# zrlhahaha/Direct12PBRRenderer

Hardware: AMD Instinct MI355X
Metric: shaded Mpixel/s at 4K G-buffer (full deferred frame: clustered shade + bloom + auto-exposure + ACES) (higher is better)
Workload: dtype f32

## Files before the change

direct12pbrrenderer_amd/_lib.py:

```python
import ctypes as C
import os

from .structs import CubeF32, GBuffer, Global, HaloPeer, Texture2D, Tile, View

_HERE = os.path.dirname(os.path.abspath(__file__))
LIB_PATH = os.environ.get("PBR_HIP_LIB", os.path.join(_HERE, "libpbr_hip.so"))

_u32, _f32, _int, _vp, _sz = C.c_uint32, C.c_float, C.c_int, C.c_void_p, C.c_size_t

SIGNATURES = {
    "pbr_version": (C.c_char_p, []),
    "pbr_cube_texels": (_sz, [_u32, _u32]),
    "pbr_cube_mip_offset": (_sz, [_u32, _u32]),
    "pbr_env_padded_texels": (_sz, [_u32, _u32]),
    "pbr_env_padded_mip_offset": (_sz, [_u32, _u32]),
    "pbr_bloom_chain_texels": (_sz, [_u32, _u32]),
    "pbr_bloom_level_offset": (_sz, [_u32, _u32, _u32]),
    "pbr_ctx_create": (_int, [_int, C.POINTER(_vp)]),
    "pbr_ctx_destroy": (None, [_vp]),
    "pbr_ctx_set_stream": (_int, [_vp, _vp]),
    "pbr_ctx_use_own_stream": (_int, [_vp]),
    "pbr_ctx_get_stream": (_vp, [_vp]),
    "pbr_ctx_side_begin": (_int, [_vp]),
    "pbr_ctx_side_end": (_int, [_vp]),
    "pbr_ctx_side_join": (_int, [_vp]),
    "pbr_last_error": (C.c_char_p, [_vp]),
    "pbr_sync": (_int, [_vp]),
    "pbr_brdf_lut": (_int, [_vp, _u32, _vp]),
    "pbr_rgbe_decode": (_int, [_vp, _vp, C.c_size_t, _vp]),
    "pbr_cube_gen_mips": (_int, [_vp, _vp, _u32, _u32]),
    "pbr_prefilter_env": (_int, [_vp, C.POINTER(CubeF32), _u32, _u32, _vp]),
    "pbr_prefilter_env_mip": (_int, [_vp, C.POINTER(CubeF32), _u32, _u32, _f32, _vp]),
    "pbr_env_pad": (_int, [_vp, _vp, _u32, _u32, _vp]),
    "pbr_sh9_project": (_int, [_vp, C.POINTER(CubeF32), _vp]),
    "pbr_cluster_build": (_int, [_vp, C.POINTER(Global), _vp]),
    "pbr_cluster_cull": (_int, [_vp, C.POINTER(Global), _vp, _int, _vp]),
    "pbr_clustered": (_int, [_vp, C.POINTER(Global), _vp, _int, _vp]),
    "pbr_deferred_shade": (_int, [_vp, C.POINTER(Global), C.POINTER(Tile), C.POINTER(GBuffer),
                                  _vp, _u32, _vp, _u32, _u32, _vp, _vp, _int, _vp, _u32]),
    "pbr_deferred_shade_rects": (_int, [_vp, C.POINTER(Global), C.POINTER(Tile), C.POINTER(GBuffer),
                                        _vp, _u32, _vp, _u32, _u32, _vp, _vp, _int, _vp, _u32, _vp, _u32]),
    "pbr_deferred_shade_f32": (_int, [_vp, C.POINTER(Global), C.POINTER(Tile), C.POINTER(GBuffer),
                                      _vp, _u32, _vp, _u32, _u32, _vp, _vp, _int, _vp, _u32]),
    "pbr_lut_fold_x": (_int, [_vp, _vp, _u32, _vp]),
    "pbr_deferred_shade_folded": (_int, [_vp, C.POINTER(Global), C.POINTER(Tile), C.POINTER(GBuffer),
                                         _vp, _u32, _vp, _u32, _u32, _vp, _vp, _int, _vp, _u32]),
    "pbr_deferred_shade_rects_folded": (_int, [_vp, C.POINTER(Global), C.POINTER(Tile), C.POINTER(GBuffer),
                                               _vp, _u32, _vp, _u32, _u32, _vp, _vp, _int, _vp, _u32, _vp, _u32]),
    "pbr_skybox": (_int, [_vp, C.POINTER(Global), C.POINTER(Tile), C.POINTER(CubeF32), _vp, _u32, _vp, _u32]),
    "pbr_gbuffer_encode": (_int, [_vp, _vp, _vp, _vp, _u32, _u32, _u32, _vp, _vp, _vp]),
    "pbr_gbuffer_raster_scratch_bytes": (_sz, [_u32, _u32, _u32]),
    "pbr_gbuffer_raster_min_scratch_bytes": (_sz, [_u32, _u32, _u32]),
    "pbr_gbuffer_raster": (_int, [_vp, C.POINTER(Global), C.POINTER(Tile), _vp, _u32, _vp, _u32, _vp, _u32, _u32,
                                  _vp, _vp, _vp, _vp, _vp, _u32, _vp, _sz]),
    "pbr_texture2d_bytes": (_sz, [_u32, _u32, _u32, _u32]),
    "pbr_bc1_decode": (_int, [_vp, _vp, _u32, _u32, _u32, _u32, _vp]),
    "pbr_bc6h_chain_bytes": (_sz, [_u32, _u32]),
    "pbr_bc6h_decode_cube": (_int, [_vp, C.POINTER(_vp * 6), _u32, _u32, _vp]),
    "pbr_texture2d_gen_mips": (_int, [_vp, _vp, _u32, _u32, _u32, _u32]),
    "pbr_bc1_encode": (_int, [_vp, _vp, _u32, _u32, _u32, _u32, _vp]),
    "pbr_gbuffer_raster_textured_scratch_bytes": (_sz, [_u32, _u32, _u32]),
    "pbr_gbuffer_raster_textured_min_scratch_bytes": (_sz, [_u32, _u32, _u32]),
    "pbr_gbuffer_raster_textured": (_int, [_vp, C.POINTER(Global), C.POINTER(Tile), _vp, _u32, _vp, _u32, _vp, _u32, _u32,
                                           _vp, _vp, _vp, _vp, _vp, _u32, _vp, _sz, _vp, C.POINTER(Texture2D), _u32]),
    "pbr_bloom_prefilter": (_int, [_vp, _vp, _u32, _u32, _u32, _vp, _f32, _f32]),
    "pbr_blur_h": (_int, [_vp, _vp, _u32, _u32, _vp, _u32, _u32]),
    "pbr_blur_v": (_int, [_vp, _vp, _u32, _u32, _vp, _u32, _u32]),
    "pbr_bloom_upsample_add": (_int, [_vp, _vp, _u32, _u32, _vp, _u32, _u32, _vp]),
    "pbr_bloom_up_level": (_int, [_vp, _vp, _vp, _u32, _u32, _vp, _u32, _u32]),
    "pbr_bloom_merge": (_int, [_vp, _vp, _u32, _vp, _u32, _u32]),
    "pbr_bloom": (_int, [_vp, _vp, _u32, _u32, _u32, _vp, _vp, _f32, _f32]),
    "pbr_bloom_prefilter_rect": (_int, [_vp, _vp, _u32, _u32, _u32, _vp, _u32, _u32, _u32, C.POINTER(_u32 * 4), _f32, _f32]),
    "pbr_bloom_prefilter_rects": (_int, [_vp, _vp, _u32, _u32, _u32, _vp, _u32, _u32, _u32, _vp, _u32, _f32, _f32]),
    "pbr_bloom_tiled": (_int, [_vp, _vp, _u32, C.POINTER(_u32 * 4), _u32, _u32, _vp, _vp, C.POINTER(_u32 * 4), _f32, _f32, _vp]),
    "pbr_bloom_histogram": (_int, [_vp, _vp, _u32, _u32, _u32, _vp, _vp, _f32, _f32, C.POINTER(_u32 * 4), _f32, _f32, _vp]),
    "pbr_lum_histogram": (_int, [_vp, _vp, _u32, _u32, _u32, _f32, _f32, _vp]),
    "pbr_lum_average": (_int, [_vp, _vp, _u32, _f32, _f32, _f32, _vp]),
    "pbr_tonemap": (_int, [_vp, _vp, _u32, _u32, _u32, _vp, _vp, _u32]),
    "pbr_average_tonemap": (_int, [_vp, _vp, _u32, _f32, _f32, _f32, _vp, _vp, _vp, _vp, _u32, _u32, _u32, _vp, _u32]),
    "pbr_clustered_views": (_int, [_vp, C.POINTER(View), _u32]),
    "pbr_deferred_shade_views": (_int, [_vp, C.POINTER(View), _u32, _u32, _u32, _vp, _u32, _vp, _u32, _u32]),
    "pbr_bloom_histogram_views": (_int, [_vp, C.POINTER(View), _u32, _u32, _u32, _f32, _f32, _f32, _f32]),
    "pbr_lum_average_views": (_int, [_vp, C.POINTER(View), _u32, _u32, _f32, _f32]),
    "pbr_tonemap_views": (_int, [_vp, C.POINTER(View), _u32, _u32, _u32]),
    "pbr_comm_unique_id": (_int, [_vp]),
    "pbr_comm_init": (_int, [_vp, _int, _int, _vp]),
    "pbr_allreduce_hist": (_int, [_vp, _vp]),
    "pbr_halo_staging_bytes": (_sz, [C.POINTER(HaloPeer), _u32]),
    "pbr_halo_exchange": (_int, [_vp, _vp, _u32, _u32, C.POINTER(HaloPeer), _u32, _vp, _sz]),
    "pbr_halo_pack": (_int, [_vp, _vp, _u32, _u32, C.POINTER(HaloPeer), _u32, _vp, _sz, _int]),
    "pbr_runtime_error": (C.c_char_p, []),
    "pbr_runtime_mismatch_dirs": (_int, [C.c_char_p, C.c_char_p]),
    "pbr_membench_read": (_int, [_vp, _vp, _sz, _vp, _u32]),
    "pbr_valubench": (_int, [_vp, _u32, _u32, _u32, _vp]),
    "pbr_ctx_set_bloom_shader_order": (_int, [_vp, _int]),
}

KNOBS_ONLY = {
    "pbr_ctx_set_cu_masks": (_int, [_vp, _vp, _vp, _u32]),
}

_lib = None


def load():
    global _lib
    if _lib is not None:
        return _lib
    if not os.path.exists(LIB_PATH):
        raise RuntimeError(
            f"{LIB_PATH} not found: build it with `make -C direct12pbrrenderer_amd/csrc` "
            "(or __graft_entry__.build()).  There is no CPU fallback for the HIP path.")
    import torch
    lib = C.CDLL(LIB_PATH)
    for name, (res, args) in SIGNATURES.items():
        fn = getattr(lib, name)
        fn.restype = res
        fn.argtypes = args
    for name, (res, args) in KNOBS_ONLY.items():
        fn = getattr(lib, name, None)
        if fn is not None:
            fn.restype = res
            fn.argtypes = args
    _lib = lib
    return lib
```

direct12pbrrenderer_amd/api.py:

```python
import ctypes as C

import numpy as np
import torch

from . import _lib
from .structs import (Texture2D, BLOOM_KNEE, BLOOM_THRESHOLD, CLUSTER_DTYPE, ENV_MIPS, HISTOGRAM_BINS,
                      INV_LOG_LUMINANCE_RANGE, LIGHT_DTYPE, LOG_LUMINANCE_RANGE, MIN_LOG_LUMINANCE,
                      NUM_CLUSTERS, DRAW_DTYPE, DRAW_MAPS_DTYPE, TEX_BC1_BLOCKS, TEX_FORMATS, VERTEX_DTYPE, CubeF32, GBuffer, Global, HaloPeer, Tile, View, bloom_chain_texels, bc6h_chain_bytes, cube_texels, env_padded_texels, texture2d_bytes)


class PbrError(RuntimeError):
    pass


def _ptr(t):
    if t is None:
        return None
    if isinstance(t, torch.Tensor):
        if not t.is_cuda:
            raise PbrError("expected a device tensor")
        if not t.is_contiguous():
            raise PbrError("expected a contiguous tensor")
        return C.c_void_p(t.data_ptr())
    return C.c_void_p(int(t))


class PbrContext:

    def __init__(self, device=0, use_torch_stream=True):
        self.lib = _lib.load()
        self.device = int(device)
        h = C.c_void_p()
        st = self.lib.pbr_ctx_create(self.device, C.byref(h))
        if st != 0:
            raise PbrError(f"pbr_ctx_create({device}) failed: status {st}")
        self.h = h
        self.torch_device = torch.device("cuda", self.device)
        if use_torch_stream:
            self.bind_torch_stream()

    def bind_torch_stream(self):
        s = torch.cuda.current_stream(self.torch_device)
        self._check(self.lib.pbr_ctx_set_stream(self.h, C.c_void_p(s.cuda_stream)))

    def close(self):
        if getattr(self, "h", None):
            self.lib.pbr_ctx_destroy(self.h)
            self.h = None

    def __del__(self):
        try:
            self.close()
        except Exception:
            pass

    def _check(self, st):
        if st != 0:
            msg = self.lib.pbr_last_error(self.h)
            raise PbrError(f"status {st}: {msg.decode() if msg else '?'}")

    def side_begin(self):
        self._check(self.lib.pbr_ctx_side_begin(self.h))

    def side_end(self):
        self._check(self.lib.pbr_ctx_side_end(self.h))

    def side_join(self):
        self._check(self.lib.pbr_ctx_side_join(self.h))

    def sync(self):
        self._check(self.lib.pbr_sync(self.h))

    def use_own_stream(self):
        self._check(self.lib.pbr_ctx_use_own_stream(self.h))

    def set_bloom_shader_order(self, on):
        self._check(self.lib.pbr_ctx_set_bloom_shader_order(self.h, 1 if on else 0))

    def partition_cus(self, side_cus, total_cus=None, layout="low", allow_uneven=False):
        if not hasattr(self.lib, "pbr_ctx_set_cu_masks"):
            raise PbrError("partition_cus: pbr_ctx_set_cu_masks is an entry point of the knobs build only (PBR_HIP_LIB=.../libpbr_hip_knobs.so): "
                           "the CU partition is a measurement aid, not part of the product library (round 6)")
        if side_cus and layout == "low" and int(side_cus) % 32 and not allow_uneven:
            raise PbrError(f"partition_cus: layout 'low' takes a multiple of 32 compute units (got {side_cus}): an uneven share per XCD runs at the poorest XCD's pace")
        if not side_cus:
            self._check(self.lib.pbr_ctx_set_cu_masks(self.h, None, None, 0))
            return
        n = int(total_cus or torch.cuda.get_device_properties(self.torch_device).multi_processor_count)
        words = (n + 31) // 32
# ... 50 lines not shown
            self._check(self.lib.pbr_prefilter_env_mip(self.h, C.byref(c), size, m, float(m) / float(max(mips - 1, 1)), C.c_void_p(dst)))
        return out

    def env_pad(self, env, size, mips=ENV_MIPS, out=None):
        out = out if out is not None else self.empty((env_padded_texels(size, mips), 4), torch.float16)
        self._check(self.lib.pbr_env_pad(self.h, _ptr(env), size, mips, _ptr(out)))
        return out

    def bc6h_decode_cube(self, faces, size, mip_levels, out=None):
        faces = list(faces)
        if len(faces) != 6:
            raise PbrError(f"bc6h_decode_cube: six faces, got {len(faces)}")
        nbytes = bc6h_chain_bytes(size, mip_levels)
        for f in faces:
            if isinstance(f, torch.Tensor) and nbytes and f.numel() * f.element_size() != nbytes:
                raise PbrError(f"bc6h_decode_cube: a face of {f.numel() * f.element_size()} bytes, {size}^2 x {mip_levels} levels takes {nbytes}")
        ptrs = (C.c_void_p * 6)(*[_ptr(f) for f in faces])
        if out is None:
            if not nbytes:
                raise PbrError(f"bad BC6H cube description: {size}^2, {mip_levels} levels")
            out = self.empty((cube_texels(size, mip_levels), 4), torch.float32)
        self._check(self.lib.pbr_bc6h_decode_cube(self.h, C.byref(ptrs), int(size), int(mip_levels), _ptr(out)))
        return out

    def sh9_project(self, sky, sky_size, sky_mips=1, out=None):
        out = out if out is not None else self.empty((28,), torch.float32)
        c = CubeF32(sky.data_ptr(), sky_size, sky_mips)
        self._check(self.lib.pbr_sh9_project(self.h, C.byref(c), _ptr(out)))
        return out

    def alloc_clusters(self):
        return self.zeros((NUM_CLUSTERS * CLUSTER_DTYPE.itemsize,), torch.uint8)

    def cluster_build(self, g: Global, clusters):
        self._check(self.lib.pbr_cluster_build(self.h, C.byref(g), _ptr(clusters)))

    def cluster_cull(self, g: Global, lights, n, clusters):
        self._check(self.lib.pbr_cluster_cull(self.h, C.byref(g), _ptr(lights), int(n), _ptr(clusters)))

    def clustered(self, g: Global, lights, n, clusters):
        self._check(self.lib.pbr_clustered(self.h, C.byref(g), _ptr(lights), int(n), _ptr(clusters)))

    def deferred_shade(self, g: Global, tile: Tile, gb, pitch, lut, lut_res, env, env_size, env_mips,
                       clusters, lights, num_lights, hdr, hdr_pitch):
        s = GBuffer(gb["A"].data_ptr(), gb["B"].data_ptr(), gb["C"].data_ptr(), gb["depth"].data_ptr(),
                    gb["stencil"].data_ptr(), pitch)
        self._check(self.lib.pbr_deferred_shade(self.h, C.byref(g), C.byref(tile), C.byref(s), _ptr(lut), lut_res,
                                                _ptr(env), env_size, env_mips, _ptr(clusters), _ptr(lights),
                                                int(num_lights), _ptr(hdr), hdr_pitch))

    @staticmethod
    def _rects(rects):
        arr = ((C.c_uint32 * 4) * len(rects))()
        for i, r in enumerate(rects):
            arr[i] = (C.c_uint32 * 4)(*[int(v) for v in r])
        return arr

    def deferred_shade_rects(self, g: Global, tile: Tile, gb, pitch, lut, lut_res, env, env_size, env_mips,
                             clusters, lights, num_lights, hdr, hdr_pitch, rects):
        s = GBuffer(gb["A"].data_ptr(), gb["B"].data_ptr(), gb["C"].data_ptr(), gb["depth"].data_ptr(),
                    gb["stencil"].data_ptr(), pitch)
        arr = self._rects(rects)
        self._check(self.lib.pbr_deferred_shade_rects(self.h, C.byref(g), C.byref(tile), C.byref(s), _ptr(lut), lut_res,
                                                      _ptr(env), env_size, env_mips, _ptr(clusters), _ptr(lights),
                                                      int(num_lights), _ptr(hdr), hdr_pitch, C.cast(arr, C.c_void_p), len(rects)))

    def lut_fold_x(self, lut, lut_res, out=None):
        out = out if out is not None else self.empty((int(lut_res), 256, 2), torch.float32)
        self._check(self.lib.pbr_lut_fold_x(self.h, _ptr(lut), int(lut_res), _ptr(out)))
        return out

    def deferred_shade_folded(self, g: Global, tile: Tile, gb, pitch, lut_fold, lut_res, env, env_size, env_mips,
                              clusters, lights, num_lights, hdr, hdr_pitch, rects=None):
        s = GBuffer(gb["A"].data_ptr(), gb["B"].data_ptr(), gb["C"].data_ptr(), gb["depth"].data_ptr(),
                    gb["stencil"].data_ptr(), pitch)
        head = (self.h, C.byref(g), C.byref(tile), C.byref(s), _ptr(lut_fold), lut_res, _ptr(env), env_size, env_mips,
                _ptr(clusters), _ptr(lights), int(num_lights), _ptr(hdr), hdr_pitch)
        if rects is None:
            self._check(self.lib.pbr_deferred_shade_folded(*head))
        else:
            arr = self._rects(rects)
            self._check(self.lib.pbr_deferred_shade_rects_folded(*head, C.cast(arr, C.c_void_p), len(rects)))

    def deferred_shade_f32(self, g: Global, tile: Tile, gb, pitch, lut, lut_res, env, env_size, env_mips,
                           clusters, lights, num_lights, hdr_f32, hdr_pitch):
        s = GBuffer(gb["A"].data_ptr(), gb["B"].data_ptr(), gb["C"].data_ptr(), gb["depth"].data_ptr(),
                    gb["stencil"].data_ptr(), pitch)
        self._check(self.lib.pbr_deferred_shade_f32(self.h, C.byref(g), C.byref(tile), C.byref(s), _ptr(lut), lut_res,
                                                    _ptr(env), env_size, env_mips, _ptr(clusters), _ptr(lights),
                                                    int(num_lights), _ptr(hdr_f32), hdr_pitch))

    def rgbe_decode(self, rgbe, out):
        self._check(self.lib.pbr_rgbe_decode(self.h, _ptr(rgbe), rgbe.numel() // 4, _ptr(out)))

    def skybox(self, g: Global, tile: Tile, sky, sky_size, sky_mips, stencil, pitch, hdr, hdr_pitch):
        c = CubeF32(sky.data_ptr(), sky_size, sky_mips)
        self._check(self.lib.pbr_skybox(self.h, C.byref(g), C.byref(tile), C.byref(c), _ptr(stencil), pitch,
                                        _ptr(hdr), hdr_pitch))

    def gbuffer_encode(self, m0, m1, m2, w, h, pitch, A, B, Cc):
        self._check(self.lib.pbr_gbuffer_encode(self.h, _ptr(m0), _ptr(m1), _ptr(m2), w, h, pitch,
                                                _ptr(A), _ptr(B), _ptr(Cc)))

    def raster_scratch_bytes(self, w, h, n_triangles, minimum=False):
        fn = self.lib.pbr_gbuffer_raster_min_scratch_bytes if minimum else self.lib.pbr_gbuffer_raster_scratch_bytes
        return int(fn(int(w), int(h), int(n_triangles)))

    def alloc_raster_scratch(self, w, h, n_triangles, minimum=False, extra=0):
        return self.empty((self.raster_scratch_bytes(w, h, n_triangles, minimum) + int(extra),), torch.uint8)

    def gbuffer_raster(self, g: Global, tile: Tile, vertices, n_vertices, indices, n_indices, draws, n_draws, max_triangles,
                       A, B, Cc, depth, stencil, pitch, scratch, scratch_bytes=None):
        nbytes = scratch.numel() * scratch.element_size() if scratch_bytes is None else int(scratch_bytes)
        self._check(self.lib.pbr_gbuffer_raster(self.h, C.byref(g), C.byref(tile), _ptr(vertices), int(n_vertices), _ptr(indices),
                                                int(n_indices), _ptr(draws), int(n_draws), int(max_triangles), _ptr(A), _ptr(B), _ptr(Cc),
                                                _ptr(depth), _ptr(stencil), int(pitch), _ptr(scratch), nbytes))

    def textured_raster_scratch_bytes(self, w, h, n_triangles, minimum=False):
        fn = self.lib.pbr_gbuffer_raster_textured_min_scratch_bytes if minimum else self.lib.pbr_gbuffer_raster_textured_scratch_bytes
        return int(fn(int(w), int(h), int(n_triangles)))

    def alloc_textured_raster_scratch(self, w, h, n_triangles, minimum=False, extra=0):
        return self.empty((self.textured_raster_scratch_bytes(w, h, n_triangles, minimum) + int(extra),), torch.uint8)

    def upload_texture(self, chain, width, height, mip_levels, fmt):
        fmt = int(fmt)
        host = np.ascontiguousarray(chain).view(np.uint8).reshape(-1)
        if fmt & TEX_BC1_BLOCKS:
            want = texture2d_bytes(width, height, mip_levels, fmt)
            if want == 0:
                raise PbrError(f"bad BC1 texture description: {width} x {height}, {mip_levels} levels, format {fmt:#x}")
            if host.size != want:
                raise PbrError(f"BC1 chain of {host.size} bytes, {width} x {height} x {mip_levels} levels takes {want}")
        elif fmt not in TEX_FORMATS:
            raise PbrError(f"unknown texture format {fmt}")
        dev = self.upload(host)
        return dev, Texture2D(dev.data_ptr(), int(width), int(height), int(mip_levels), fmt)

    def bc1_decode(self, blocks, width, height, mip_levels, stored_format, out=None):
        if isinstance(blocks, tuple):
            blocks = blocks[0]
        nbytes = texture2d_bytes(width, height, mip_levels, int(stored_format))
        if nbytes == 0 or int(stored_format) & TEX_BC1_BLOCKS:
            raise PbrError(f"bad texture description: {width} x {height}, {mip_levels} levels, stored format {stored_format}")
        if blocks.numel() * blocks.element_size() != texture2d_bytes(width, height, mip_levels, int(stored_format) | TEX_BC1_BLOCKS):
            raise PbrError("bc1_decode: the block tensor's size does not match the description")
        out = out if out is not None else self.empty((nbytes,), torch.uint8)
        self._check(self.lib.pbr_bc1_decode(self.h, _ptr(blocks), int(width), int(height), int(mip_levels), int(stored_format), _ptr(out)))
        return out, Texture2D(out.data_ptr(), int(width), int(height), int(mip_levels), int(stored_format))

    def texture2d_gen_mips(self, chain, width, height, mip_levels, fmt):
        if isinstance(chain, tuple):
            chain = chain[0]
        nbytes = texture2d_bytes(width, height, mip_levels, int(fmt))
        if nbytes == 0 or int(fmt) & TEX_BC1_BLOCKS:
            raise PbrError(f"bad texture description: {width} x {height}, {mip_levels} levels, format {fmt}")
        if chain.numel() * chain.element_size() != nbytes:
            raise PbrError("texture2d_gen_mips: the chain tensor's size does not match the description")
        self._check(self.lib.pbr_texture2d_gen_mips(self.h, _ptr(chain), int(width), int(height), int(mip_levels), int(fmt)))

    def bc1_encode(self, texels, width, height, mip_levels, stored_format, out=None):
        if isinstance(texels, tuple):
            texels = texels[0]
        fmt = int(stored_format)
        nbytes = texture2d_bytes(width, height, mip_levels, fmt | TEX_BC1_BLOCKS)
        if nbytes == 0 or fmt & TEX_BC1_BLOCKS:
# ... 163 lines not shown
```

direct12pbrrenderer_amd/csrc/cluster.hip:

```cpp
#include "pbr_internal.hpp"
#include "pbr_device.hpp"
#include <type_traits>

using namespace pbr;

struct ClusterParams {
    float Near, Far, Ratio, Fov;
    float View[12];
};

__device__ __forceinline__ int cluster_index3(int x, int y, int z) {
    return z + x * PBR_CLUSTER_Z + y * PBR_CLUSTER_X * PBR_CLUSTER_Z;
}

__device__ __forceinline__ void cluster_bounds(const ClusterParams& p, int t, float mn[3], float mx[3]) {
    const int z = t % PBR_CLUSTER_Z, tx = (t / PBR_CLUSTER_Z) % PBR_CLUSTER_X, ty = t / (PBR_CLUSTER_Z * PBR_CLUSTER_X);
    const float htan = tanf(p.Fov / 2.0f);
    const float znear = p.Near * powf(p.Far / p.Near, (float)z / (float)PBR_CLUSTER_Z);
    const float zfar = p.Near * powf(p.Far / p.Near, (float)(z + 1) / (float)PBR_CLUSTER_Z);
    const float minx = 2.0f * (float)tx / (float)PBR_CLUSTER_X - 1.0f, miny = 2.0f * (float)ty / (float)PBR_CLUSTER_Y - 1.0f;
    const float maxx = 2.0f * (float)(tx + 1) / (float)PBR_CLUSTER_X - 1.0f, maxy = 2.0f * (float)(ty + 1) / (float)PBR_CLUSTER_Y - 1.0f;
    auto zplane = [&](float nx, float ny, float vz) {
        V3 ray = v3(nx * p.Ratio * htan, ny * htan, 1.0f) * p.Near;
        float tt = vz / ray.z;
        return ray * tt;
    };
    V3 min_near = zplane(minx, miny, znear), min_far = zplane(minx, miny, zfar);
    V3 max_near = zplane(maxx, maxy, znear), max_far = zplane(maxx, maxy, zfar);
    mn[0] = fminf(min_near.x, min_far.x); mn[1] = fminf(min_near.y, min_far.y); mn[2] = fminf(min_near.z, min_far.z);
    mx[0] = fmaxf(max_near.x, max_far.x); mx[1] = fmaxf(max_near.y, max_far.y); mx[2] = fmaxf(max_near.z, max_far.z);
}

__global__ __launch_bounds__(256) void k_cluster_build(ClusterParams p, pbr_cluster* __restrict__ clusters) {
    const int t = blockIdx.x * 256 + threadIdx.x;
    if (t >= PBR_NUM_CLUSTERS) return;
    float mn[3], mx[3];
    cluster_bounds(p, t, mn, mx);
    pbr_cluster* c = clusters + t;
    c->MinBound[0] = mn[0]; c->MinBound[1] = mn[1]; c->MinBound[2] = mn[2];
    c->MaxBound[0] = mx[0]; c->MaxBound[1] = mx[1]; c->MaxBound[2] = mx[2];
    c->NumLights = 0;
}

__device__ __forceinline__ bool light_hits(const ClusterParams& p, const pbr_light& l, const float* mn, const float* mx) {
#pragma clang fp contract(off)
    const float px = ((p.View[0] * l.Position[0] + p.View[1] * l.Position[1]) + p.View[2] * l.Position[2]) + p.View[3];
    const float py = ((p.View[4] * l.Position[0] + p.View[5] * l.Position[1]) + p.View[6] * l.Position[2]) + p.View[7];
    const float pz = ((p.View[8] * l.Position[0] + p.View[9] * l.Position[1]) + p.View[10] * l.Position[2]) + p.View[11];
    const float radius = l.Radius * 1.814f * sqrtf(l.Intensity);
    const float dx = px - fminf(fmaxf(px, mn[0]), mx[0]);
    const float dy = py - fminf(fmaxf(py, mn[1]), mx[1]);
    const float dz = pz - fminf(fmaxf(pz, mn[2]), mx[2]);
    return (dx * dx + dy * dy) + dz * dz < radius * radius;
}

struct ClusterView {
    ClusterParams p;
    const pbr_light* lights;
    int n;
    pbr_cluster* clusters;
};
struct ClusterViews { ClusterView v[PBR_MAX_VIEWS]; };
static_assert(sizeof(ClusterViews) <= 4096 - 256, "k_cluster_cull<.., ClusterViews>: kernel arguments over 4 KiB");

template <bool BUILD, class VS = NoViews>
__global__ __launch_bounds__(256) void k_cluster_cull(ClusterParams p_, const pbr_light* __restrict__ lights_, int n_, VS vs,
                                                        pbr_cluster* __restrict__ clusters_) {
    constexpr bool MV = !std::is_same_v<VS, NoViews>;
    const ClusterView* view = nullptr;
    if constexpr (MV) view = &vs.v[blockIdx.y];
    const ClusterParams& p = MV ? view->p : p_;
    const pbr_light* __restrict__ lights = MV ? view->lights : lights_;
    const int n = MV ? view->n : n_;
    pbr_cluster* __restrict__ clusters = MV ? view->clusters : clusters_;
    const int lane = threadIdx.x & 63;
    const int ci = blockIdx.x * 4 + (threadIdx.x >> 6);
    if (ci >= PBR_NUM_CLUSTERS) return;
    pbr_cluster* c = clusters + ci;
    float mn[3], mx[3];
    int count = 0;
    if (BUILD) {
        cluster_bounds(p, ci, mn, mx);
        if (lane < 3) { c->MinBound[lane] = mn[lane]; c->MaxBound[lane] = mx[lane]; }
    } else {
        mn[0] = c->MinBound[0]; mn[1] = c->MinBound[1]; mn[2] = c->MinBound[2];
        mx[0] = c->MaxBound[0]; mx[1] = c->MaxBound[1]; mx[2] = c->MaxBound[2];
        count = c->NumLights;
        count = min(max(count, 0), PBR_MAX_LIGHTS_PER_CLUSTER);
    }
    for (int base = 0; base < n && count < PBR_MAX_LIGHTS_PER_CLUSTER; base += 64) {
        const int i = base + lane;
        bool hit = false;
        if (i < n) hit = light_hits(p, lights[i], mn, mx);
        const unsigned long long mask = __ballot(hit);
        const int pos = count + __popcll(mask & ((1ull << lane) - 1ull));
        if (hit && pos < PBR_MAX_LIGHTS_PER_CLUSTER) c->LightIndex[pos] = i;
        count = min(count + __popcll(mask), PBR_MAX_LIGHTS_PER_CLUSTER);
    }
    if (lane == 0) c->NumLights = count;
}

static ClusterParams make_params(const pbr_global* g) {
    ClusterParams p;
    p.Near = g->Near; p.Far = g->Far; p.Ratio = g->Ratio; p.Fov = g->Fov;
    for (int i = 0; i < 12; i++) p.View[i] = g->View[i];
    return p;
}

static const char* cull_args_bad(const pbr_global* g, bool build, const pbr_light* lights, int n) {
    if (build && !(g->Near > 0.0f && g->Far > g->Near)) return "need 0 < Near < Far";
    if (!(n >= 0 && n <= PBR_MAX_SCENE_LIGHTS)) return "light count out of [0, 1024]";
    if (!(n == 0 || lights != nullptr)) return "null lights";
    return nullptr;
}

extern "C" {

pbr_status pbr_cluster_build(pbr_ctx* ctx, const pbr_global* g, pbr_cluster* clusters) {
    if (!ctx) return PBR_ERR_INVALID;
    PBR_REQUIRE(ctx, g && clusters, "pbr_cluster_build: null pointer");
    PBR_REQUIRE(ctx, g->Near > 0.0f && g->Far > g->Near, "pbr_cluster_build: need 0 < Near < Far");
    hipLaunchKernelGGL(k_cluster_build, dim3(PBR_NUM_CLUSTERS / 256), dim3(256), 0, ctx->stream, make_params(g), clusters);
    return launched(ctx, "k_cluster_build");
}

pbr_status pbr_cluster_cull(pbr_ctx* ctx, const pbr_global* g, const pbr_light* lights, int n, pbr_cluster* clusters) {
    if (!ctx) return PBR_ERR_INVALID;
    PBR_REQUIRE(ctx, g && clusters, "pbr_cluster_cull: null pointer");
    PBR_CHECK(ctx, "pbr_cluster_cull", cull_args_bad(g, false, lights, n));
    if (n == 0) return PBR_OK;
    hipLaunchKernelGGL(k_cluster_cull<false>, dim3(PBR_NUM_CLUSTERS / 4), dim3(256), 0, ctx->stream, make_params(g), lights, n, NoViews{}, clusters);
    return launched(ctx, "k_cluster_cull");
}

pbr_status pbr_clustered(pbr_ctx* ctx, const pbr_global* g, const pbr_light* lights, int n, pbr_cluster* clusters) {
    if (!ctx) return PBR_ERR_INVALID;
    PBR_REQUIRE(ctx, g && clusters, "pbr_clustered: null pointer");
    PBR_CHECK(ctx, "pbr_clustered", cull_args_bad(g, true, lights, n));
    hipLaunchKernelGGL(k_cluster_cull<true>, dim3(PBR_NUM_CLUSTERS / 4), dim3(256), 0, ctx->stream, make_params(g), lights, n, NoViews{}, clusters);
    return launched(ctx, "k_cluster_cull<build>");
}

pbr_status pbr_clustered_views(pbr_ctx* ctx, const pbr_view* views, uint32_t n) {
    if (!ctx) return PBR_ERR_INVALID;
    PBR_REQUIRE(ctx, views_count_ok(views, n), "pbr_clustered_views: need 1 .. PBR_MAX_VIEWS views");
    ClusterViews vs{};
    for (uint32_t i = 0; i < n; i++) {
        const pbr_view& v = views[i];
        PBR_REQUIRE(ctx, v.clusters, "pbr_clustered_views: null clusters");
        PBR_CHECK(ctx, "pbr_clustered_views", cull_args_bad(&v.g, true, v.lights, v.num_lights));
        vs.v[i] = ClusterView{make_params(&v.g), v.lights, v.num_lights, v.clusters};
    }
    PBR_REQUIRE(ctx, views_disjoint(views, n, 1, [](const pbr_view& v, int, uintptr_t& lo, uintptr_t& hi) {
                    lo = addr(v.clusters); hi = lo + (size_t)PBR_NUM_CLUSTERS * sizeof(pbr_cluster); }),
                "pbr_clustered_views: two views share a cluster buffer");
    hipLaunchKernelGGL((k_cluster_cull<true, ClusterViews>), dim3(PBR_NUM_CLUSTERS / 4, n), dim3(256), 0, ctx->stream,
                       ClusterParams{}, (const pbr_light*)nullptr, 0, vs, (pbr_cluster*)nullptr);
    return launched(ctx, "k_cluster_cull<views>");
}

}
```

direct12pbrrenderer_amd/csrc/pbr_device.hpp:

```cpp
#pragma once
#include <hip/hip_runtime.h>
#include <stdint.h>
#include "../../include/pbr_hip.h"

namespace pbr {

constexpr float PI_F = 3.14159265359f;
constexpr float INV_PI_F = 0.31830988618f;
constexpr float EPSILON_F = 1e-6f;
constexpr float TWO_PI_F = (float)(2.0 * 3.14159265359);

typedef _Float16 h16;

struct V3 { float x, y, z; };
__device__ __forceinline__ V3 v3(float x, float y, float z) { return V3{x, y, z}; }
__device__ __forceinline__ V3 operator+(V3 a, V3 b) { return v3(a.x + b.x, a.y + b.y, a.z + b.z); }
__device__ __forceinline__ V3 operator-(V3 a, V3 b) { return v3(a.x - b.x, a.y - b.y, a.z - b.z); }
__device__ __forceinline__ V3 operator*(V3 a, V3 b) { return v3(a.x * b.x, a.y * b.y, a.z * b.z); }
__device__ __forceinline__ V3 operator*(V3 a, float s) { return v3(a.x * s, a.y * s, a.z * s); }
__device__ __forceinline__ float dot3(V3 a, V3 b) { return a.x * b.x + a.y * b.y + a.z * b.z; }
__device__ __forceinline__ V3 cross3(V3 a, V3 b) {
    return v3(a.y * b.z - a.z * b.y, a.z * b.x - a.x * b.z, a.x * b.y - a.y * b.x);
}
__device__ __forceinline__ float rsq(float x) { return __builtin_amdgcn_rsqf(x); }
__device__ __forceinline__ float rcp(float x) { return __builtin_amdgcn_rcpf(x); }
__device__ __forceinline__ V3 normalize3(V3 v) { return v * rsq(dot3(v, v)); }
__device__ __forceinline__ V3 normalize3_exact(V3 v) { return v * (1.0f / sqrtf(dot3(v, v))); }
__device__ __forceinline__ float saturatef(float x) { return __builtin_amdgcn_fmed3f(x, 0.0f, 1.0f); }
__device__ __forceinline__ int clampi(int v, int lo, int hi) { return min(max(v, lo), hi); }

struct F4 { float x, y, z, w; };
__device__ __forceinline__ F4 f4(float x, float y, float z, float w) { return F4{x, y, z, w}; }
__device__ __forceinline__ F4 operator+(F4 a, F4 b) { return f4(a.x + b.x, a.y + b.y, a.z + b.z, a.w + b.w); }
__device__ __forceinline__ F4 operator*(F4 a, float s) { return f4(a.x * s, a.y * s, a.z * s, a.w * s); }

struct alignas(8) H4 { h16 x, y, z, w; };
__device__ __forceinline__ F4 load_h4(const pbr_half* p) {
    H4 h = *reinterpret_cast<const H4*>(p);
    return f4((float)h.x, (float)h.y, (float)h.z, (float)h.w);
}
__device__ __forceinline__ h16 to_half_rn(float v) {
    asm volatile("" : "+v"(v));
    return (h16)v;
}
__device__ __forceinline__ void store_h4(pbr_half* p, F4 v) {
    H4 h;
    h.x = to_half_rn(v.x); h.y = to_half_rn(v.y); h.z = to_half_rn(v.z); h.w = to_half_rn(v.w);
    *reinterpret_cast<H4*>(p) = h;
}
struct alignas(4) H2 { h16 x, y; };

struct BilinearCoord { int i0, i1; float f; };
__device__ __forceinline__ float snap8(float x) { return floorf(x * 256.0f + 0.5f) * (1.0f / 256.0f); }
__device__ __forceinline__ BilinearCoord bilinear_coord(float u, int size) {
    float c = u * (float)size;
    c = (c == c) ? c : 0.5f;
    c = fminf(fmaxf(c, -1.5f), (float)size + 1.5f);
    float x = snap8(c) - 0.5f;
    float fl = floorf(x);
    BilinearCoord b;
    b.i0 = (int)fl;
    b.i1 = b.i0 + 1;
    b.f = x - fl;
    return b;
}
__device__ __forceinline__ F4 fma4(F4 a, float s, F4 b) {
    return f4(__builtin_fmaf(a.x, s, b.x), __builtin_fmaf(a.y, s, b.y), __builtin_fmaf(a.z, s, b.z), __builtin_fmaf(a.w, s, b.w));
}
__device__ __forceinline__ F4 lerp4(F4 a, F4 b, float f) {
    const F4 r = fma4(b, f, a * (1.0f - f));
    return f == 0.0f ? a : r;
}
__device__ __forceinline__ F4 bilerp(F4 c00, F4 c10, F4 c01, F4 c11, float fx, float fy) {
    return lerp4(lerp4(c00, c10, fx), lerp4(c01, c11, fx), fy);
}
__device__ __forceinline__ F4 sample_2d_h4(const pbr_half* img, int w, int h, int pitch, float u, float v) {
    BilinearCoord cx = bilinear_coord(u, w), cy = bilinear_coord(v, h);
    int x0 = clampi(cx.i0, 0, w - 1), x1 = clampi(cx.i1, 0, w - 1);
    int y0 = clampi(cy.i0, 0, h - 1), y1 = clampi(cy.i1, 0, h - 1);
    F4 c00 = load_h4(img + 4 * ((size_t)y0 * pitch + x0));
    F4 c10 = load_h4(img + 4 * ((size_t)y0 * pitch + x1));
    F4 c01 = load_h4(img + 4 * ((size_t)y1 * pitch + x0));
    F4 c11 = load_h4(img + 4 * ((size_t)y1 * pitch + x1));
    return bilerp(c00, c10, c01, c11, cx.f, cy.f);
}

__device__ __forceinline__ V3 cube_dir_raw(uint32_t face, float u, float v) {
    switch (face) {
        case 0: return v3(1.0f, -v, -u);
        case 1: return v3(-1.0f, -v, u);
        case 2: return v3(u, 1.0f, v);
        case 3: return v3(u, -1.0f, -v);
        case 4: return v3(u, -v, 1.0f);
        default: return v3(-u, -v, -1.0f);
    }
// ... 136 lines not shown
```

direct12pbrrenderer_amd/csrc/shade.hip:

```cpp
#include <cstring>
#include <type_traits>
#include "pbr_internal.hpp"
#include "pbr_device.hpp"

using namespace pbr;

struct ShadeParams {
    pbr_sh_pack sh;
    float InvView[9];
    float CameraPos[3];
    float Near, Far;
    float near_width, near_height;
    float log_far_near;
    float inv_near, slice_k;
    uint32_t x0, y0, w, h, full_w, full_h;
    const uint32_t* A;
    const uint32_t* B;
    const uint32_t* C;
    const float* depth;
    const uint8_t* stencil;
    uint32_t pitch;
    const pbr_half* lut;
    const float* lut_fold;
    uint32_t lut_res;
    const pbr_half* env;
    uint32_t env_size, env_mips;
    uint32_t env_mip_off[16];
    const pbr_cluster* clusters;
    const pbr_light* lights;
    pbr_half* hdr;
    uint32_t hdr_pitch;
    float* hdr_f32;
};

__device__ __forceinline__ float view_space_depth(float d, float near_z, float far_z) {
#pragma clang fp contract(off)
    const float range = far_z - near_z;
    const float prod = d * range;
    const float den = far_z - prod;
    const float num = near_z * far_z;
    return num / den;
}

__device__ __forceinline__ float view_space_depth_quick(float d, float near_z, float far_z) {
#pragma clang fp contract(off)
    const float range = far_z - near_z;
    const float prod = d * range;
    const float den = far_z - prod;
    return (near_z * far_z) * rcp(den);
}

__device__ __forceinline__ float sign_custom(float x) { return x < 0.0f ? -1.0f : 1.0f; }

__device__ __forceinline__ V3 decode_octahedron(float u, float v) {
    V3 d = v3(u * 2.0f - 1.0f, v * 2.0f - 1.0f, 0.0f);
    d.z = 1.0f - fabsf(d.x) - fabsf(d.y);
    if (d.z < 0.0f) {
        float nx = sign_custom(d.x) * (1.0f - fabsf(d.y));
        float ny = sign_custom(d.y) * (1.0f - fabsf(d.x));
        d.x = nx; d.y = ny;
    }
    return d;
}

__global__ __launch_bounds__(256) void k_env_pad(const pbr_half* __restrict__ src, pbr_half* __restrict__ dst, int s) {
    const int sq = s + 1;
    const size_t n = (size_t)6 * sq * sq * 4;
    const size_t t = (size_t)blockIdx.x * 256 + threadIdx.x;
    if (t >= n) return;
    const int k = (int)(t & 3), xq = (int)((t >> 2) % sq), yq = (int)(((t >> 2) / sq) % sq);
    uint32_t face = (uint32_t)((t >> 2) / ((size_t)sq * sq));
    int x = xq - 1 + (k & 1), y = yq - 1 + (k >> 1);
    const bool xo = (x < 0) | (x >= s), yo = (y < 0) | (y >= s);
    if (xo | yo) {
        if (xo & yo) y = clampi(y, 0, s - 1);
        const float uu = 2.0f * ((float)x + 0.5f) / (float)s - 1.0f;
        const float vv = 2.0f * ((float)y + 0.5f) / (float)s - 1.0f;
        float u2, v2;
        cube_face_uv(cube_dir_raw(face, uu, vv), face, u2, v2);
        x = clampi((int)floorf(u2 * (float)s), 0, s - 1);
        y = clampi((int)floorf(v2 * (float)s), 0, s - 1);
    }
    reinterpret_cast<H4*>(dst)[t] = reinterpret_cast<const H4*>(src)[((size_t)face * s + y) * s + x];
}

constexpr int LIGHT_PLANES = 9;

constexpr int SHADE_MAX_RECTS = 5;
struct ShadeRects {
    uint32_t n, rows_big, rows_small;
    uint32_t x0[SHADE_MAX_RECTS], y0[SHADE_MAX_RECTS], w[SHADE_MAX_RECTS], h[SHADE_MAX_RECTS];
    uint32_t cols[SHADE_MAX_RECTS], nb_big[SHADE_MAX_RECTS], first[SHADE_MAX_RECTS + 1];
};

constexpr int SHADE_BLOCK = 256;
constexpr int SHADE_ROWS = 8;
constexpr int MAX_STAGED_TILES = 12;
constexpr int LIST_STRIDE = 34;
#ifndef SHADE_WALK_TRIPS
#define SHADE_WALK_TRIPS 2
#endif
constexpr int WALK_TRIPS = SHADE_WALK_TRIPS;
static_assert(WALK_TRIPS == 2 || WALK_TRIPS == 4, "a staging thread converts four entries: the padded length must be a multiple of four that divides 32");

typedef float f2 __attribute__((ext_vector_type(2)));
__device__ __forceinline__ f2 f2s(float a) { return f2{a, a}; }
__device__ __forceinline__ f2 max2(f2 a, f2 b) { return f2{fmaxf(a.x, b.x), fmaxf(a.y, b.y)}; }
typedef __attribute__((address_space(3))) const float lds_cf;
__device__ __forceinline__ f2 rsq2(f2 a) { return f2{rsq(a.x), rsq(a.y)}; }
__device__ __forceinline__ f2 rcp2(f2 a) { return f2{rcp(a.x), rcp(a.y)}; }

__device__ __forceinline__ f2 mul2_sat(f2 a, f2 b) {
    f2 r;
    asm("s_nop 0\n\tv_pk_mul_f32 %0, %1, %2 clamp\n\ts_nop 0" : "=v"(r) : "v"(a), "v"(b));
    return r;
}

__device__ __forceinline__ f2 zero2() {
    f2 r;
    asm("v_pk_mov_b32 %0, 0, 0\n\ts_nop 0" : "=v"(r));
    return r;
}

struct alignas(8) H4x2 { H4 a, b; };
struct alignas(4) H2x2 { H2 a, b; };

struct LutX { int xb; float fx, wx0; };
__device__ __forceinline__ LutX lut_x_side(float roughness, int lr) {
    const float xs = snap8(roughness * (float)lr) - 0.5f;
    const float xfl = floorf(xs);
    const int xi = (int)xfl;
    LutX r;
    r.xb = clampi(xi, 0, max(lr - 2, 0));
    r.fx = xi < 0 ? 0.0f : (xi > lr - 2 ? 1.0f : xs - xfl);
    r.wx0 = 1.0f - r.fx;
    return r;
}
__device__ __forceinline__ H2x2 lut_row_pair(const pbr_half* lut_, int lr, int y, int xb) {
    const H2* lut = reinterpret_cast<const H2*>(lut_);
    H2x2 lt;
    if (lr > 1) lt = *reinterpret_cast<const H2x2*>(reinterpret_cast<const char*>(lut) + (__umul24((uint32_t)y, (uint32_t)lr) + (uint32_t)xb) * 4u);
    else lt.a = lt.b = lut[0];
    return lt;
}
__device__ __forceinline__ float lut_x_lerp(h16 a, h16 b, const LutX& x) { return __builtin_fmaf((float)b, x.fx, __builtin_fmaf((float)a, x.wx0, 0.0f)); }

__global__ __launch_bounds__(256) void k_lut_fold_x(const pbr_half* __restrict__ lut, int lr, float* __restrict__ out) {
    const uint32_t t = blockIdx.x * 256u + threadIdx.x;
    const int y = (int)(t >> 8);
    if (y >= lr) return;
    const float roughness = (float)(t & 255u) * (1.0f / 255.0f);
    const LutX x = lut_x_side(roughness, lr);
    const H2x2 lt = lut_row_pair(lut, lr, y, x.xb);
    reinterpret_cast<float2*>(out)[t] = make_float2(lut_x_lerp(lt.a.x, lt.b.x, x), lut_x_lerp(lt.a.y, lt.b.y, x));
}

template <bool STAGED_LISTS, int LSTRIDE, bool F32OUT, bool LUTFOLD>
__device__ __forceinline__ void shade_pixel(const ShadeParams& p, const float* llds, const uint32_t* lists, const uint32_t* mip_off,
                                            int n_lights, int q_safe, uint32_t px, uint32_t py, float4 row, float cvv_x, uint32_t col_list) {
    const uint32_t gi = __umul24(py, p.pitch) + px;
    auto at = [](const auto* base, uint32_t byte_off) { return *reinterpret_cast<std::remove_reference_t<decltype(*base)>*>(reinterpret_cast<const char*>(base) + byte_off); };
    if (at(p.stencil, gi) == 0) return;
    const float inv255 = 1.0f / 255.0f;

    V3 pos, view, n;
    float z_vs, roughness, depth_keep;
    {
        const uint32_t b = at(p.B, gi * 4u), c = at(p.C, gi * 4u);
        const float depth_ndc = at(p.depth, gi * 4u);
        const V3 camera_vec = v3(__builtin_fmaf(p.InvView[2], p.Near, __builtin_fmaf(p.InvView[0], cvv_x, row.x)),
                                 __builtin_fmaf(p.InvView[5], p.Near, __builtin_fmaf(p.InvView[3], cvv_x, row.y)),
                                 __builtin_fmaf(p.InvView[8], p.Near, __builtin_fmaf(p.InvView[6], cvv_x, row.z)));
        roughness = (float)(c & 255u) * inv255;
        n = normalize3(decode_octahedron((float)(b & 255u) * inv255, (float)((b >> 8) & 255u) * inv255));
        z_vs = view_space_depth_quick(depth_ndc, p.Near, p.Far);
        depth_keep = depth_ndc;
        const V3 cam = v3(p.CameraPos[0], p.CameraPos[1], p.CameraPos[2]);
        const float zs = z_vs * p.inv_near;
        pos = v3(cam.x + camera_vec.x * zs, cam.y + camera_vec.y * zs, cam.z + camera_vec.z * zs);
        view = normalize3(cam - pos);
    }
    const float NdV = dot3(n, view);
    const float NdotV = fmaxf(NdV, 0.0f);

// ... 291 lines not shown
        llds[1 * LSTRIDE + i] = l.Position[1];
        llds[2 * LSTRIDE + i] = l.Position[2];
        llds[3 * LSTRIDE + i] = l.Color[0] * l.Intensity;
        llds[4 * LSTRIDE + i] = l.Color[1] * l.Intensity;
        llds[5 * LSTRIDE + i] = l.Color[2] * l.Intensity;
        llds[6 * LSTRIDE + i] = l.C0;
        llds[7 * LSTRIDE + i] = l.C1;
        llds[8 * LSTRIDE + i] = l.C2;
    }
    uint32_t r = 0;
    while (r + 1 < rc.n && blockIdx.x >= rc.first[r + 1]) r++;
    const uint32_t lb = blockIdx.x - rc.first[r];
    const uint32_t bx0 = rc.x0[r] + (lb % rc.cols[r]) * SHADE_BLOCK, x_end = rc.x0[r] + rc.w[r];
    const uint32_t by = lb / rc.cols[r], nb_big = rc.nb_big[r], rows_big = rc.rows_big, rows_small = rc.rows_small;
    const uint32_t y_begin = rc.y0[r] + (by < nb_big ? by * rows_big : nb_big * rows_big + (by - nb_big) * rows_small);
    const uint32_t y_end = min(y_begin + (by < nb_big ? rows_big : rows_small), rc.y0[r] + rc.h[r]);
    int tile_x0 = 0, tile_y0 = 0, tiles_x = 1;
    const uint32_t lds_base = (uint32_t)(uintptr_t)(lds_cf*)llds;
    if (STAGED_LISTS) {
        const uint32_t bx1 = min(bx0 + SHADE_BLOCK, x_end) - 1;
        auto tx = [&](uint32_t x) { return clampi((int)floorf((((float)(p.x0 + x) + 0.5f) / (float)p.full_w) * (float)PBR_CLUSTER_X), 0, PBR_CLUSTER_X - 1); };
        auto ty = [&](uint32_t y) { return clampi((int)floorf((1.0f - ((float)(p.y0 + y) + 0.5f) / (float)p.full_h) * (float)PBR_CLUSTER_Y), 0, PBR_CLUSTER_Y - 1); };
        tile_x0 = tx(bx0);
        const int tile_x1 = tx(bx1);
        const int ty_a = ty(y_begin), ty_b = ty(y_end - 1);
        tile_y0 = min(ty_a, ty_b);
        const int tile_y1 = max(ty_a, ty_b);
        tiles_x = tile_x1 - tile_x0 + 1;
        const int n_cl = min(tiles_x * (tile_y1 - tile_y0 + 1) * PBR_CLUSTER_Z, max_clusters);
        {
            static_assert(PBR_CLUSTER_Z == 8 && PBR_MAX_LIGHTS_PER_CLUSTER == 32, "staging map");
            struct __attribute__((packed, aligned(4))) Idx4 { int32_t x, y, z, w; };
            const int part = threadIdx.x & 7;
            const float inv_tiles_x = rcp((float)tiles_x);
            for (int c = threadIdx.x >> 3; c < n_cl; c += SHADE_BLOCK / 8) {
                const int z = c & 7, t = c >> 3;
                const int ty_ = (int)(((float)t + 0.5f) * inv_tiles_x), cx = tile_x0 + (t - ty_ * tiles_x), cy = tile_y0 + ty_;
                const pbr_cluster* cl = p.clusters + (z + cx * PBR_CLUSTER_Z + cy * PBR_CLUSTER_X * PBR_CLUSTER_Z);
                const int cnt = n_lights > 0 ? min(max(cl->NumLights, 0), PBR_MAX_LIGHTS_PER_CLUSTER) : 0;
                const Idx4 v = *reinterpret_cast<const Idx4*>(cl->LightIndex + 4 * part);
                uint32_t* l = lists + c * LIST_STRIDE;
                const int padded = max((cnt + 2 * WALK_TRIPS - 1) & ~(2 * WALK_TRIPS - 1), 2 * WALK_TRIPS);
                if (4 * part < padded) {
                    auto entry = [&](int k, int raw) { return lds_base + 4u * (uint32_t)(4 * part + k < cnt ? min(max(raw, 0), n_lights - 1) : n_lights); };
                    uint2* e = reinterpret_cast<uint2*>(l + 2 + 4 * part);
                    e[0] = make_uint2(entry(0, v.x), entry(1, v.y));
                    e[1] = make_uint2(entry(2, v.z), entry(3, v.w));
                }
                if (part == 0) *reinterpret_cast<uint2*>(l) = make_uint2((uint32_t)padded, 0u);
            }
        }
    }
    __shared__ float4 s_row[SHADE_ROWS];
    if (threadIdx.x < (uint32_t)SHADE_ROWS) {
        const float v = ((float)(p.y0 + y_begin + threadIdx.x) + 0.5f) / (float)p.full_h;
        const float ndc_y = 1.0f - 2.0f * v;
        const float cvv_y = ndc_y * 0.5f * p.near_height;
        const int sy = clampi((int)floorf((1.0f - v) * (float)PBR_CLUSTER_Y), 0, PBR_CLUSTER_Y - 1);
        const uint32_t row_list = STAGED_LISTS ? (uint32_t)((sy - tile_y0) * tiles_x * (PBR_CLUSTER_Z * LIST_STRIDE)) : (uint32_t)(sy * (PBR_CLUSTER_X * PBR_CLUSTER_Z));
        s_row[threadIdx.x] = make_float4(p.InvView[1] * cvv_y, p.InvView[4] * cvv_y, p.InvView[7] * cvv_y, __uint_as_float(row_list));
    }
    const int q_safe = (__syncthreads_and(my_safe) != 0 ? 1 : 0) | (__syncthreads_and(my_same) != 0 ? 2 : 0);
    SHADE_ISTAMP(blockIdx.x, 0, t_start);
    SHADE_ISTAMP(blockIdx.x, 1, SHADE_NOW());
    SHADE_ISTAMP(blockIdx.x, 3, ((unsigned long long)(y_end - y_begin) << 48) | blockIdx.x);
    const uint32_t px = bx0 + threadIdx.x;
    const float u = ((float)(p.x0 + px) + 0.5f) / (float)p.full_w;
    const float ndc_x = 2.0f * u - 1.0f;
    const float cvv_x = ndc_x * 0.5f * p.near_width;
    const int sx = clampi((int)floorf(u * (float)PBR_CLUSTER_X), 0, PBR_CLUSTER_X - 1);
    const uint32_t col_list = STAGED_LISTS ? (uint32_t)((sx - tile_x0) * (PBR_CLUSTER_Z * LIST_STRIDE)) : (uint32_t)(sx * PBR_CLUSTER_Z);
#ifndef PBR_SHADE_TIMING
    if (px >= x_end) return;
    for (uint32_t py = y_begin; py < y_end; py++)
        shade_pixel<STAGED_LISTS, LSTRIDE, F32OUT, LUTFOLD>(p, llds, lists, s_mip_off, n_lights, q_safe, px, py, s_row[py - y_begin], cvv_x, col_list);
#else
    if (px < x_end)
        for (uint32_t py = y_begin; py < y_end; py++)
            shade_pixel<STAGED_LISTS, LSTRIDE, F32OUT, LUTFOLD>(p, llds, lists, s_mip_off, n_lights, q_safe, px, py, s_row[py - y_begin], cvv_x, col_list);
    SHADE_ISTAMP_MAX(blockIdx.x, 2, SHADE_NOW());
#endif
}

extern "C" {

pbr_status pbr_env_pad(pbr_ctx* ctx, const pbr_half* env, uint32_t size, uint32_t mips, pbr_half* out_padded) {
    if (!ctx) return PBR_ERR_INVALID;
    PBR_REQUIRE(ctx, env && out_padded, "pbr_env_pad: null pointer");
    PBR_REQUIRE(ctx, size >= 1 && size <= 8192 && mips >= 1 && mips <= 16 && (size >> (mips - 1)) >= 1, "pbr_env_pad: bad size/mips");
    for (uint32_t m = 0; m < mips; m++) {
        const int s = (int)(size >> m);
        const size_t n = (size_t)6 * (s + 1) * (s + 1) * 4;
        hipLaunchKernelGGL(k_env_pad, dim3((unsigned)((n + 255) / 256)), dim3(256), 0, ctx->stream,
                           env + 4 * cube_mip_offset(size, m), out_padded + 4 * env_padded_mip_offset(size, m), s);
        pbr_status r = launched(ctx, "k_env_pad");
        if (r) return r;
    }
    return PBR_OK;
}

}

static void camera_params(const pbr_global* g, ShadeParams& p) {
    p.sh = g->SkyBoxSH;
    for (int r = 0; r < 3; r++)
        for (int c = 0; c < 3; c++) p.InvView[r * 3 + c] = g->InvView[r * 4 + c];
    for (int i = 0; i < 3; i++) p.CameraPos[i] = g->CameraPos[i];
    p.Near = g->Near; p.Far = g->Far;
    p.near_height = 2.0f * g->Near * tanf(g->Fov / 2.0f);
    p.near_width = p.near_height * g->Ratio;
    p.log_far_near = logf(g->Far / g->Near);
    p.inv_near = (float)(1.0 / (double)g->Near);
    p.slice_k = (float)((double)PBR_CLUSTER_Z / log2((double)g->Far / (double)g->Near));
}

static ShadeParams shade_params(const pbr_global* g, const pbr_half* lut, uint32_t lut_res, const pbr_half* env, uint32_t env_size, uint32_t env_mips) {
    ShadeParams p{};
    camera_params(g, p);
    p.lut = lut; p.lut_res = lut_res; p.env = env; p.env_size = env_size; p.env_mips = env_mips;
    for (uint32_t m = 0; m < 16; m++) p.env_mip_off[m] = (uint32_t)env_padded_mip_offset(env_size, m < env_mips ? m : env_mips - 1);
    return p;
}

static const char* shade_tables_bad(const void* lut, uint32_t lut_res, const pbr_half* env, uint32_t env_size, uint32_t env_mips, uint32_t lut_align = 4) {
    if (!lut || !env) return "null pointer";
    if (!(lut_res >= 1 && env_size >= 1 && env_mips >= 1 && env_mips <= 16 && (env_size >> (env_mips - 1)) >= 1)) return "bad LUT/env size";
    if (!(lut_res <= 16384 && (uint64_t)pbr_env_padded_texels(env_size, env_mips) * 8u < (1ull << 32)))
        return "LUT larger than 16384^2 or padded env chain of 4 GiB or more (32-bit texture offsets)";
    if (((uintptr_t)env & 7u) != 0 || ((uintptr_t)lut & (lut_align - 1u)) != 0) return lut_align == 4 ? "env must be 8-byte and lut 4-byte aligned" : "env and the folded LUT must be 8-byte aligned";
    return nullptr;
}

static const char* shade_target_bad(const pbr_global* g, const pbr_gbuffer& gb, const pbr_cluster* clusters, const void* out, uint32_t out_pitch,
                                    uint32_t w, uint32_t h, const pbr_light* lights, int num_lights) {
    if (!clusters || !out) return "null pointer";
    if (!(gb.A && gb.B && gb.C && gb.depth && gb.stencil)) return "null G-buffer plane";
    if (!(gb.pitch >= w && out_pitch >= w)) return "pitch < width";
    if (!((uint64_t)gb.pitch * h * 4u < (1ull << 32) && (uint64_t)out_pitch * h * 16u < (1ull << 32)))
        return "target too large for 32-bit plane offsets (pitch x rows x 16 bytes must stay below 4 GiB)";
    if (!(g->Near > 0.0f && g->Far > g->Near)) return "need 0 < Near < Far";
    if (!(num_lights >= 0 && num_lights <= PBR_MAX_SCENE_LIGHTS)) return "light count out of [0, 1024]";
    if (!(num_lights == 0 || lights != nullptr)) return "null lights";
    return nullptr;
}

static ShadeRects shade_schedule(const pbr_ctx* ctx, const uint32_t (*rects)[4], uint32_t n_rects, uint32_t n_views) {
    static const float big_frac = pbr::knob_float("PBR_SHADE_BIGFRAC", 0.92f);
    static const uint32_t rows_small_cfg = (uint32_t)pbr::knob_int("PBR_SHADE_ROWS_SMALL", 1);
    static const uint32_t rows_big_cfg = (uint32_t)pbr::knob_int("PBR_SHADE_ROWS_BIG", 0);
    const uint32_t rows_small = rows_small_cfg >= 1 && rows_small_cfg <= (uint32_t)SHADE_ROWS ? rows_small_cfg : 1u;
    uint64_t row_segments = 0;
    for (uint32_t r = 0; r < n_rects; r++) row_segments += (uint64_t)((rects[r][2] + SHADE_BLOCK - 1) / SHADE_BLOCK) * rects[r][3];
    row_segments *= n_views;
    uint32_t rows_big = (uint32_t)SHADE_ROWS;
    const uint64_t slots = (uint64_t)ctx->cu_count * SHADE_MIN_WAVES;
    if (row_segments * 10 < slots * 13 * SHADE_ROWS) {
        const uint32_t rws = (uint32_t)((row_segments * 10 + slots * 8) / (slots * 16));
        rows_big = rws < 2 ? 2u : (rws > (uint32_t)SHADE_ROWS ? (uint32_t)SHADE_ROWS : rws);
    }
    if (rows_big_cfg >= 1 && rows_big_cfg <= (uint32_t)SHADE_ROWS) rows_big = rows_big_cfg;
    ShadeRects rc{};
    rc.n = n_rects; rc.rows_big = rows_big; rc.rows_small = rows_small < rows_big ? rows_small : rows_big;
    uint32_t blocks = 0;
    for (uint32_t r = 0; r < n_rects; r++) {
        const uint32_t* q = rects[r];
        rc.x0[r] = q[0]; rc.y0[r] = q[1]; rc.w[r] = q[2]; rc.h[r] = q[3];
        rc.cols[r] = (q[2] + SHADE_BLOCK - 1) / SHADE_BLOCK;
        rc.nb_big[r] = (uint32_t)((float)(q[3] / rows_big) * fminf(fmaxf(big_frac, 0.0f), 1.0f));
        const uint32_t rest = q[3] - rc.nb_big[r] * rows_big;
        rc.first[r] = blocks;
        blocks += rc.cols[r] * (rc.nb_big[r] + (rest + rc.rows_small - 1) / rc.rows_small);
    }
    rc.first[n_rects] = blocks;
    return rc;
}

template <bool F32OUT, bool LUTFOLD, class VS>
static pbr_status shade_dispatch(pbr_ctx* ctx, const ShadeParams& p, int num_lights, int max_lights, const ShadeRects& rc, uint32_t n_views, const VS& vs) {
    const uint32_t span_x = (uint32_t)((uint64_t)(SHADE_BLOCK - 1) * PBR_CLUSTER_X / p.full_w) + 2;
    const uint32_t span_y = (uint32_t)((uint64_t)(SHADE_ROWS - 1) * PBR_CLUSTER_Y / p.full_h) + 2;
    const int lstride = max_lights <= 256 ? 257 : PBR_MAX_SCENE_LIGHTS + 1;
    const size_t plane_bytes = (size_t)((LIGHT_PLANES * lstride + 1) & ~1) * sizeof(float);
    const bool staged = span_x * span_y <= (uint32_t)MAX_STAGED_TILES &&
                        plane_bytes + (size_t)span_x * span_y * PBR_CLUSTER_Z * LIST_STRIDE * sizeof(uint32_t) <= 65536;
    const int max_clusters = staged ? (int)(span_x * span_y) * PBR_CLUSTER_Z : 0;
    const size_t lds = plane_bytes + (size_t)max_clusters * LIST_STRIDE * sizeof(uint32_t);
    const dim3 grid(rc.first[rc.n], n_views), blk(SHADE_BLOCK);
    if (staged && lstride == 257) hipLaunchKernelGGL((k_deferred_shade<true, 257, F32OUT, VS, LUTFOLD>), grid, blk, lds, ctx->stream, p, num_lights, max_clusters, rc, vs);
    else if (staged) hipLaunchKernelGGL((k_deferred_shade<true, PBR_MAX_SCENE_LIGHTS + 1, F32OUT, VS, LUTFOLD>), grid, blk, lds, ctx->stream, p, num_lights, max_clusters, rc, vs);
    else if (lstride == 257) hipLaunchKernelGGL((k_deferred_shade<false, 257, F32OUT, VS, LUTFOLD>), grid, blk, lds, ctx->stream, p, num_lights, 0, rc, vs);
    else hipLaunchKernelGGL((k_deferred_shade<false, PBR_MAX_SCENE_LIGHTS + 1, F32OUT, VS, LUTFOLD>), grid, blk, lds, ctx->stream, p, num_lights, 0, rc, vs);
    return launched(ctx, std::is_same_v<VS, NoViews> ? "k_deferred_shade" : "k_deferred_shade<views>");
}

template <bool F32OUT, bool LUTFOLD = false>
static pbr_status shade_launch(pbr_ctx* ctx, const pbr_global* g, const pbr_tile* tile, const pbr_gbuffer* gb,
                               const void* lut, uint32_t lut_res,
                               const pbr_half* env, uint32_t env_size, uint32_t env_mips,
                               const pbr_cluster* clusters, const pbr_light* lights, int num_lights,
                               pbr_half* hdr, float* hdr_f32, uint32_t hdr_pitch,
                               const uint32_t (*rects)[4] = nullptr, uint32_t n_rects = 0) {
    if (!ctx) return PBR_ERR_INVALID;
    const char* who = "pbr_deferred_shade";
    PBR_REQUIRE(ctx, g && tile && gb, "pbr_deferred_shade: null pointer");
    PBR_REQUIRE(ctx, tile->w >= 1 && tile->h >= 1 && tile->w <= 65535 && tile->h <= 65535, "pbr_deferred_shade: bad tile size");
    PBR_REQUIRE(ctx, tile->x0 + tile->w <= tile->full_w && tile->y0 + tile->h <= tile->full_h, "pbr_deferred_shade: tile outside frame");
    PBR_CHECK(ctx, who, shade_target_bad(g, *gb, clusters, F32OUT ? (const void*)hdr_f32 : (const void*)hdr, hdr_pitch, tile->w, tile->h, lights, num_lights));
    PBR_CHECK(ctx, who, shade_tables_bad(lut, lut_res, env, env_size, env_mips, LUTFOLD ? 8 : 4));
    const uint32_t whole[1][4] = {{0, 0, tile->w, tile->h}};
    if (!rects) { rects = whole; n_rects = 1; }
    PBR_REQUIRE(ctx, n_rects >= 1 && n_rects <= (uint32_t)SHADE_MAX_RECTS, "pbr_deferred_shade: 1 .. 5 rectangles");
    for (uint32_t r = 0; r < n_rects; r++) {
        const uint32_t* q = rects[r];
        PBR_REQUIRE(ctx, q[2] >= 1 && q[3] >= 1 && q[0] + q[2] <= tile->w && q[1] + q[3] <= tile->h, "pbr_deferred_shade: rectangle outside the tile");
    }
    ShadeParams p = shade_params(g, LUTFOLD ? nullptr : (const pbr_half*)lut, lut_res, env, env_size, env_mips);
    if (LUTFOLD) p.lut_fold = (const float*)lut;
    p.x0 = tile->x0; p.y0 = tile->y0; p.w = tile->w; p.h = tile->h; p.full_w = tile->full_w; p.full_h = tile->full_h;
    p.A = gb->A; p.B = gb->B; p.C = gb->C; p.depth = gb->depth; p.stencil = gb->stencil; p.pitch = gb->pitch;
    p.clusters = clusters; p.lights = lights; p.hdr = hdr; p.hdr_pitch = hdr_pitch; p.hdr_f32 = hdr_f32;
    return shade_dispatch<F32OUT, LUTFOLD>(ctx, p, num_lights, num_lights, shade_schedule(ctx, rects, n_rects, 1), 1, NoViews{});
}

extern "C" {

pbr_status pbr_deferred_shade(pbr_ctx* ctx, const pbr_global* g, const pbr_tile* tile, const pbr_gbuffer* gb,
                              const pbr_half* lut, uint32_t lut_res,
                              const pbr_half* env, uint32_t env_size, uint32_t env_mips,
                              const pbr_cluster* clusters, const pbr_light* lights, int num_lights,
                              pbr_half* hdr, uint32_t hdr_pitch) {
    return shade_launch<false>(ctx, g, tile, gb, lut, lut_res, env, env_size, env_mips, clusters, lights, num_lights, hdr, nullptr, hdr_pitch);
}

pbr_status pbr_deferred_shade_rects(pbr_ctx* ctx, const pbr_global* g, const pbr_tile* tile, const pbr_gbuffer* gb,
                                    const pbr_half* lut, uint32_t lut_res,
                                    const pbr_half* env, uint32_t env_size, uint32_t env_mips,
                                    const pbr_cluster* clusters, const pbr_light* lights, int num_lights,
                                    pbr_half* hdr, uint32_t hdr_pitch, const uint32_t (*rects)[4], uint32_t n_rects) {
    if (ctx && !rects) return pbr::fail(ctx, PBR_ERR_INVALID, "pbr_deferred_shade_rects: null rectangle list");
    return shade_launch<false>(ctx, g, tile, gb, lut, lut_res, env, env_size, env_mips, clusters, lights, num_lights, hdr, nullptr, hdr_pitch, rects, n_rects);
}

pbr_status pbr_lut_fold_x(pbr_ctx* ctx, const pbr_half* lut, uint32_t lut_res, float* out_fold) {
    if (!ctx) return PBR_ERR_INVALID;
    PBR_REQUIRE(ctx, lut && out_fold, "pbr_lut_fold_x: null pointer");
    PBR_REQUIRE(ctx, lut_res >= 1 && lut_res <= 16384, "pbr_lut_fold_x: lut_res out of [1, 16384]");
    PBR_REQUIRE(ctx, ((uintptr_t)lut & 3u) == 0 && ((uintptr_t)out_fold & 7u) == 0, "pbr_lut_fold_x: lut must be 4-byte and the table 8-byte aligned");
    hipLaunchKernelGGL(k_lut_fold_x, dim3(lut_res), dim3(256), 0, ctx->stream, lut, (int)lut_res, out_fold);
    return launched(ctx, "k_lut_fold_x");
}

pbr_status pbr_deferred_shade_folded(pbr_ctx* ctx, const pbr_global* g, const pbr_tile* tile, const pbr_gbuffer* gb,
                                     const float* lut_fold, uint32_t lut_res,
                                     const pbr_half* env, uint32_t env_size, uint32_t env_mips,
                                     const pbr_cluster* clusters, const pbr_light* lights, int num_lights,
                                     pbr_half* hdr, uint32_t hdr_pitch) {
    return shade_launch<false, true>(ctx, g, tile, gb, lut_fold, lut_res, env, env_size, env_mips, clusters, lights, num_lights, hdr, nullptr, hdr_pitch);
}

pbr_status pbr_deferred_shade_rects_folded(pbr_ctx* ctx, const pbr_global* g, const pbr_tile* tile, const pbr_gbuffer* gb,
                                           const float* lut_fold, uint32_t lut_res,
                                           const pbr_half* env, uint32_t env_size, uint32_t env_mips,
                                           const pbr_cluster* clusters, const pbr_light* lights, int num_lights,
                                           pbr_half* hdr, uint32_t hdr_pitch, const uint32_t (*rects)[4], uint32_t n_rects) {
    if (ctx && !rects) return pbr::fail(ctx, PBR_ERR_INVALID, "pbr_deferred_shade_rects_folded: null rectangle list");
    return shade_launch<false, true>(ctx, g, tile, gb, lut_fold, lut_res, env, env_size, env_mips, clusters, lights, num_lights, hdr, nullptr, hdr_pitch, rects, n_rects);
}

pbr_status pbr_deferred_shade_f32(pbr_ctx* ctx, const pbr_global* g, const pbr_tile* tile, const pbr_gbuffer* gb,
                                  const pbr_half* lut, uint32_t lut_res,
                                  const pbr_half* env, uint32_t env_size, uint32_t env_mips,
                                  const pbr_cluster* clusters, const pbr_light* lights, int num_lights,
                                  float* hdr_f32, uint32_t hdr_pitch) {
    if (ctx && hdr_f32 && ((uintptr_t)hdr_f32 & 15u) != 0) return pbr::fail(ctx, PBR_ERR_INVALID, "pbr_deferred_shade_f32: output must be 16-byte aligned");
    return shade_launch<true>(ctx, g, tile, gb, lut, lut_res, env, env_size, env_mips, clusters, lights, num_lights, nullptr, hdr_f32, hdr_pitch);
}

pbr_status pbr_deferred_shade_views(pbr_ctx* ctx, const pbr_view* views, uint32_t n, uint32_t w, uint32_t h,
                                    const pbr_half* lut, uint32_t lut_res,
                                    const pbr_half* env, uint32_t env_size, uint32_t env_mips) {
    if (!ctx) return PBR_ERR_INVALID;
    const char* who = "pbr_deferred_shade_views";
    PBR_REQUIRE(ctx, views_count_ok(views, n), "pbr_deferred_shade_views: need 1 .. PBR_MAX_VIEWS views");
    PBR_REQUIRE(ctx, w >= 1 && h >= 1 && w <= 65535 && h <= 65535, "pbr_deferred_shade_views: bad frame size");
    PBR_CHECK(ctx, who, shade_tables_bad(lut, lut_res, env, env_size, env_mips));
    ShadeViews vs{};
    int max_lights = 0;
    for (uint32_t i = 0; i < n; i++) {
        const pbr_view& v = views[i];
        PBR_CHECK(ctx, who, shade_target_bad(&v.g, v.gb, v.clusters, v.hdr, v.hdr_pitch, w, h, v.lights, v.num_lights));
        PBR_REQUIRE(ctx, memcmp(&v.g.SkyBoxSH, &views[0].g.SkyBoxSH, sizeof(pbr_sh_pack)) == 0, "pbr_deferred_shade_views: SkyBoxSH differs between views");
        ShadeParams c;
        camera_params(&v.g, c);
        ShadeView& d = vs.v[i];
        for (int k = 0; k < 9; k++) d.InvView[k] = c.InvView[k];
        for (int k = 0; k < 3; k++) d.CameraPos[k] = c.CameraPos[k];
        d.Near = c.Near; d.Far = c.Far; d.near_width = c.near_width; d.near_height = c.near_height;
        d.log_far_near = c.log_far_near; d.inv_near = c.inv_near; d.slice_k = c.slice_k;
        d.A = v.gb.A; d.B = v.gb.B; d.C = v.gb.C; d.depth = v.gb.depth; d.stencil = v.gb.stencil; d.pitch = v.gb.pitch;
        d.clusters = v.clusters; d.lights = v.lights; d.hdr = v.hdr; d.hdr_pitch = v.hdr_pitch; d.n_lights = v.num_lights;
        max_lights = v.num_lights > max_lights ? v.num_lights : max_lights;
    }
    PBR_REQUIRE(ctx, views_disjoint(views, n, 1, [&](const pbr_view& v, int, uintptr_t& lo, uintptr_t& hi) {
                    lo = addr(v.hdr); hi = lo + ((size_t)v.hdr_pitch * (h - 1) + w) * 8u; }),
                "pbr_deferred_shade_views: two views share an HDR target");
    ShadeParams p = shade_params(&views[0].g, lut, lut_res, env, env_size, env_mips);
    p.w = p.full_w = w; p.h = p.full_h = h;
    const uint32_t whole[1][4] = {{0, 0, w, h}};
    return shade_dispatch<false, false>(ctx, p, 0, max_lights, shade_schedule(ctx, whole, 1, n), n, vs);
}

}
```

direct12pbrrenderer_amd/host/HipCommandList.cpp:

```cpp
#include "HipCommandList.h"

#include "ShaderConstants.h"

#include <dlfcn.h>

namespace MRendererHip {

static const std::vector<ShaderReflection>& Reflections() {
    static const std::vector<ShaderReflection> table = {
        {"precompute_brdf.hlsl", true, {}, {"PrecomputeBRDF"}, {}, {}, sizeof(PrecomputeBRDFConstant)},
        {"env_map_gen.hlsl", true, {"SkyBox"}, {"PrefilterEnvMap"}, {}, {}, sizeof(PreFilterEnvMapConstant)},
        {"clustered_compute.hlsl", true, {}, {}, {}, {"Clusters"}, sizeof(ClusteredShaderConstant)},
        {"clustered_culling.hlsl", true, {}, {}, {}, {"Clusters", "PointLights"}, sizeof(ClusteredShaderConstant)},
        {"deferred_shading.hlsl", false,
         {"GBufferA", "GBufferB", "GBufferC", "DepthStencil", "PrecomputeBRDF", "PrefilterEnvMap"}, {}, {"Clusters", "PointLights"}, {}, 0},
        {"bloom_prefilter.hlsl", true, {"InputTexture"}, {"OutputTexture"}, {}, {}, sizeof(BloomPrefilterConstant)},
        {"blur_horizontal.hlsl", true, {"InputTexture"}, {"OutputTexture"}, {}, {}, sizeof(BlurConstant)},
        {"blur_vertical.hlsl", true, {"InputTexture"}, {"OutputTexture"}, {}, {}, sizeof(BlurConstant)},
        {"bloom_upsample_add.hlsl", true, {"UpperLevel", "LowerLevel"}, {"OutputTexture"}, {}, {}, sizeof(BlurConstant)},
        {"bloom_merge.hlsl", true, {"InputTexture"}, {"OutputTexture"}, {}, {}, 0},
        {"hdr_luminance_histogram.hlsl", true, {"LuminanceTexture"}, {}, {}, {"LuminanceHistogram"}, sizeof(LuminanceHistogramConstant)},
        {"hdr_average_histogram.hlsl", true, {}, {}, {}, {"LuminanceHistogram", "AverageLuminance"}, sizeof(AverageLuminanceConstant)},
        {"hdr_tone_mapping.hlsl", false, {"LuminanceTexture"}, {}, {}, {"AverageLuminance"}, 0},
        {"gbuffer.hlsl", false, {}, {}, {}, {}, 0},
// ... 168 lines not shown
                if (!n) return false;
                *offset = off;
                *bytes = n;
                return true;
            }
            off += n;
        }
    return false;
}

namespace {
struct Roctx {
    int (*push)(const char*) = nullptr;
    int (*pop)() = nullptr;
    Roctx() {
        void* h = nullptr;
        const char* names[] = {"libroctx64.so.4", "libroctx64.so", "/opt/rocm/lib/libroctx64.so.4"};
        for (const char* n : names) if ((h = dlopen(n, RTLD_NOW | RTLD_NOLOAD))) break;
        if (!h) for (const char* n : names) if ((h = dlopen(n, RTLD_NOW | RTLD_GLOBAL))) break;
        if (!h) return;
        push = (int (*)(const char*))dlsym(h, "roctxRangePushA");
        pop = (int (*)())dlsym(h, "roctxRangePop");
        if (!push || !pop) push = nullptr, pop = nullptr;
    }
};
const Roctx& roctx() { static const Roctx r; return r; }
}
void HipCommandList::BeginEvent(const char* name) {
    mEventLog.emplace_back(name);
    if (roctx().push) roctx().push(name);
}
void HipCommandList::EndEvent() {
    if (roctx().pop) roctx().pop();
}
void HipCommandList::SetExternalHistogram(const uint32* counts256) {
    if (counts256) mExternalHistogram.assign(counts256, counts256 + 256);
    else mExternalHistogram.clear();
}

namespace {
struct Mip {
    pbr_half* ptr;
    uint32 w, h;
};
Mip MipOf(const TextureBinding& b) {
    auto* t = dynamic_cast<DeviceTexture2D*>(b.Texture);
    if (!t) throw HipException("expected a 2D texture binding");
    uint32 m = b.MipSlice < 0 ? 0 : (uint32)b.MipSlice;
    return Mip{(pbr_half*)t->MipPtr(m), t->Width() >> m, t->Height() >> m};
}
uint32 Groups(uint32 size, uint32 group) { return (size + group - 1) / group; }
void ExpectGroups(std::string_view file, uint32 gx, uint32 gy, uint32 gz, uint32 ex, uint32 ey, uint32 ez) {
    if (gx != ex || gy != ey || gz != ez)
        throw HipException(std::string(file) + ": dispatch shape (" + std::to_string(gx) + "," + std::to_string(gy) + "," + std::to_string(gz) +
                           ") does not cover the bound output (" + std::to_string(ex) + "," + std::to_string(ey) + "," + std::to_string(ez) + ")");
}
}

void HipCommandList::Dispatch(ShadingState* s, uint32 gx, uint32 gy, uint32 gz) {
    if (!s || !s->GetShader() || !s->IsCompute()) throw HipException("Dispatch: shading state has no compute shader");
    const std::string_view f = s->File();
    mDispatchCount++;
    if (f != "hdr_luminance_histogram.hlsl") FlushPendingBloom();
    if (f == "precompute_brdf.hlsl") {
        const auto& c = s->Constants<PrecomputeBRDFConstant>();
        auto* out = dynamic_cast<DeviceTexture2D*>(s->RWTexture("PrecomputeBRDF").Texture);
        if (!out || out->Width() != c.TextureResolution || out->Height() != c.TextureResolution) throw HipException("precompute_brdf: LUT size != TextureResolution");
        ExpectGroups(f, gx, gy, gz, Groups(c.TextureResolution, 8), Groups(c.TextureResolution, 8), 1);
        Check(pbr_brdf_lut(mCtx, c.TextureResolution, (pbr_half*)out->DevicePtr()), "pbr_brdf_lut");
        mFoldedLut.erase(out);
    } else if (f == "env_map_gen.hlsl") {
        const auto& c = s->Constants<PreFilterEnvMapConstant>();
        auto* sky = dynamic_cast<DeviceTexture2DArray*>(s->Texture("SkyBox").Texture);
        auto* out = dynamic_cast<DeviceTexture2DArray*>(s->RWTexture("PrefilterEnvMap").Texture);
        if (!sky || !out || out->Size() != c.EnvMapSize || c.MipLevel >= out->MipLevels()) throw HipException("env_map_gen: bad bindings");
        const uint32 ms = c.EnvMapSize >> c.MipLevel;
        ExpectGroups(f, gx, gy, gz, Groups(ms, 8), Groups(ms, 8), 6);
        pbr_cube_f32 cube{(const float*)sky->DevicePtr(), sky->Size(), sky->MipLevels()};
        pbr_half* dst = (pbr_half*)out->DevicePtr() + 4 * pbr_cube_mip_offset(out->Size(), c.MipLevel);
        Check(pbr_prefilter_env_mip(mCtx, &cube, c.EnvMapSize, c.MipLevel, c.Roughness, dst), "pbr_prefilter_env_mip");
        mPaddedEnv.erase(out);
    } else if (f == "clustered_compute.hlsl") {
        ExpectGroups(f, gx, gy, gz, 1, 1, 1);
        Check(pbr_cluster_build(mCtx, &mGlobal, (pbr_cluster*)s->Buffer("Clusters")->DevicePtr()), "pbr_cluster_build");
    } else if (f == "clustered_culling.hlsl") {
        ExpectGroups(f, gx, gy, gz, 1, 1, 1);
        const auto& c = s->Constants<ClusteredShaderConstant>();
        mNumLights = c.NumLight;
        Check(pbr_cluster_cull(mCtx, &mGlobal, (const pbr_light*)s->Buffer("PointLights")->DevicePtr(), c.NumLight,
                               (pbr_cluster*)s->Buffer("Clusters")->DevicePtr()), "pbr_cluster_cull");
    } else if (f == "bloom_prefilter.hlsl") {
        if (mTailOverlap == 2) BeginTail();
        const auto& c = s->Constants<BloomPrefilterConstant>();
        Mip in = MipOf(s->Texture("InputTexture")), out = MipOf(s->RWTexture("OutputTexture"));
        ExpectGroups(f, gx, gy, gz, Groups(in.w, 16), Groups(in.h, 16), 1);
        if (out.w != (in.w >> 1) || out.h != (in.h >> 1)) throw HipException("bloom_prefilter: output is not the half-res mip");
        Check(pbr_bloom_prefilter(mCtx, in.ptr, in.w, in.h, in.w, out.ptr, c.Threshold, c.Knee), "pbr_bloom_prefilter");
    } else if (f == "blur_horizontal.hlsl" || f == "blur_vertical.hlsl") {
        Mip in = MipOf(s->Texture("InputTexture")), out = MipOf(s->RWTexture("OutputTexture"));
        (void)s->Constants<BlurConstant>();
        if (f == "blur_horizontal.hlsl") {
            ExpectGroups(f, gx, gy, gz, Groups(out.w, 256), out.h, 1);
            Check(pbr_blur_h(mCtx, in.ptr, in.w, in.h, out.ptr, out.w, out.h), "pbr_blur_h");
        } else {
            ExpectGroups(f, gx, gy, gz, out.w, Groups(out.h, 256), 1);
            Check(pbr_blur_v(mCtx, in.ptr, in.w, in.h, out.ptr, out.w, out.h), "pbr_blur_v");
        }
    } else if (f == "bloom_upsample_add.hlsl") {
        Mip up = MipOf(s->Texture("UpperLevel")), lo = MipOf(s->Texture("LowerLevel")), out = MipOf(s->RWTexture("OutputTexture"));
        ExpectGroups(f, gx, gy, gz, Groups(out.w, 256), out.h, 1);
        if (out.w != up.w || out.h != up.h) throw HipException("bloom_upsample_add: output size != upper level");
        Check(pbr_bloom_upsample_add(mCtx, up.ptr, up.w, up.h, lo.ptr, lo.w, lo.h, out.ptr), "pbr_bloom_upsample_add");
    } else if (f == "bloom_merge.hlsl") {
        Mip in = MipOf(s->Texture("InputTexture")), out = MipOf(s->RWTexture("OutputTexture"));
        ExpectGroups(f, gx, gy, gz, Groups(out.w, 16), Groups(out.h, 16), 1);
        Check(pbr_bloom_merge(mCtx, out.ptr, out.w, in.ptr, out.w, out.h), "pbr_bloom_merge");
    } else if (f == "hdr_luminance_histogram.hlsl") {
        const auto& c = s->Constants<LuminanceHistogramConstant>();
        Mip in = MipOf(s->Texture("LuminanceTexture"));
        ExpectGroups(f, gx, gy, gz, Groups(c.TextureWidth, 16), Groups(c.TextureHeight, 16), 1);
        uint32_t* hist = (uint32_t*)s->Buffer("LuminanceHistogram")->DevicePtr();
        const Rect r = mInterior.w ? mInterior : Rect{0, 0, in.w, in.h};
        if (r.x + r.w > in.w || r.y + r.h > in.h || c.TextureWidth != r.w || c.TextureHeight != r.h)
            throw HipException("hdr_luminance_histogram: TextureWidth/Height must be the interior rectangle's size");
        const TextureBinding& lum = s->Texture("LuminanceTexture");
        if (mPendingBloom.What != PendingBloom::None && lum.Texture == mPendingBloom.Hdr && lum.MipSlice <= 0) {
            FlushPendingBloom(hist, c.MinLogLuminance, c.InvLogLuminanceRange);
        } else {
            FlushPendingBloom();
            Check(pbr_lum_histogram(mCtx, in.ptr + 4 * ((size_t)r.y * in.w + r.x), r.w, r.h, in.w, c.MinLogLuminance, c.InvLogLuminanceRange, hist),
                  "pbr_lum_histogram");
        }
        if (mCaptureHistogram) {
            Check(pbr_sync(mCtx), "pbr_sync");
            mCapturedHistogram.resize(256);
            ThrowIfFailed(hipMemcpy(mCapturedHistogram.data(), hist, 1024, hipMemcpyDeviceToHost), "read histogram");
        }
    } else if (f == "hdr_average_histogram.hlsl") {
        const auto& c = s->Constants<AverageLuminanceConstant>();
        ExpectGroups(f, gx, gy, gz, 1, 1, 1);
        uint32_t* hist = (uint32_t*)s->Buffer("LuminanceHistogram")->DevicePtr();
        BeginTail();
        Check(pbr_allreduce_hist(mCtx, hist), "pbr_allreduce_hist");
        if (!mExternalHistogram.empty()) {
            Check(pbr_sync(mCtx), "pbr_sync");
            std::vector<uint32> mine(256);
            ThrowIfFailed(hipMemcpy(mine.data(), hist, 1024, hipMemcpyDeviceToHost), "read histogram");
            for (int i = 0; i < 256; i++) mine[i] += mExternalHistogram[i];
            ThrowIfFailed(hipMemcpy(hist, mine.data(), 1024, hipMemcpyHostToDevice), "write histogram");
        }
        Check(pbr_lum_average(mCtx, hist, c.PixelCount, c.MinLogLuminance, c.LogLuminanceRange, mGlobal.DeltaTime,
                              (float*)s->Buffer("AverageLuminance")->DevicePtr()), "pbr_lum_average");
    } else {
        throw HipException("Dispatch: " + std::string(f) + " is not a compute kernel of this build");
    }
}

void HipCommandList::DrawScreen(ShadingState* s) {
    if (!s || !s->GetShader() || s->IsCompute()) throw HipException("DrawScreen: shading state has no pixel shader");
    const std::string_view f = s->File();
    mDispatchCount++;
    FlushPendingBloom();
    if (!mRenderTarget) throw HipException("DrawScreen: no render target bound (FrameGraph::PreparePass)");
    if (f == "deferred_shading.hlsl") {
        auto tex = [&](const char* n) { return dynamic_cast<DeviceTexture2D*>(s->Texture(n).Texture); };
        DeviceTexture2D *a = tex("GBufferA"), *b = tex("GBufferB"), *c = tex("GBufferC"), *ds = tex("DepthStencil"), *lut = tex("PrecomputeBRDF");
        auto* env = dynamic_cast<DeviceTexture2DArray*>(s->Texture("PrefilterEnvMap").Texture);
        if (!a || !b || !c || !ds || !lut || !env) throw HipException("deferred_shading: bad texture bindings");
        const uint32 w = mRenderTarget->Width(), h = mRenderTarget->Height();
        pbr_gbuffer gb{(const uint32_t*)a->DevicePtr(), (const uint32_t*)b->DevicePtr(), (const uint32_t*)c->DevicePtr(),
                       ds->DepthPlane(), ds->StencilPlane(), w};
        pbr_tile tile = mTile.w ? mTile : pbr_tile{0, 0, w, h, w, h};
        auto& padded = mPaddedEnv[env];
        if (!padded) {
            padded = std::make_unique<DeviceStructuredBuffer>((uint32)(pbr_env_padded_texels(env->Size(), env->MipLevels()) * 8), 8);
            Check(pbr_env_pad(mCtx, (const pbr_half*)env->DevicePtr(), env->Size(), env->MipLevels(), (pbr_half*)padded->DevicePtr()), "pbr_env_pad");
        }
        auto& folded = mFoldedLut[lut];
        if (!folded) {
            folded = std::make_unique<DeviceStructuredBuffer>(lut->Width() * 256u * 8u, 8);
            Check(pbr_lut_fold_x(mCtx, (const pbr_half*)lut->DevicePtr(), lut->Width(), (float*)folded->DevicePtr()), "pbr_lut_fold_x");
        }
        if (mStencilRef != 0) throw HipException("deferred_shading: only stencil ref 0 is supported");
        Check(pbr_deferred_shade_folded(mCtx, &mGlobal, &tile, &gb, (const float*)folded->DevicePtr(), lut->Width(),
                                        (const pbr_half*)padded->DevicePtr(), env->Size(), env->MipLevels(),
                                        (const pbr_cluster*)s->Buffer("Clusters")->DevicePtr(), (const pbr_light*)s->Buffer("PointLights")->DevicePtr(),
                                        mNumLights, (pbr_half*)mRenderTarget->DevicePtr(), w), "pbr_deferred_shade_folded");
    } else if (f == "hdr_tone_mapping.hlsl") {
        Mip in = MipOf(s->Texture("LuminanceTexture"));
        const Rect r = mInterior.w ? mInterior : Rect{0, 0, in.w, in.h};
        if (r.x + r.w > in.w || r.y + r.h > in.h || mRenderTarget->Width() < in.w) throw HipException("hdr_tone_mapping: interior rectangle outside the target");
        Check(pbr_tonemap(mCtx, in.ptr + 4 * ((size_t)r.y * in.w + r.x), r.w, r.h, in.w, (const float*)s->Buffer("AverageLuminance")->DevicePtr(),
                          (uint32_t*)mRenderTarget->DevicePtr() + (size_t)r.y * mRenderTarget->Width() + r.x, mRenderTarget->Width()), "pbr_tonemap");
        EndTail();
    } else {
        throw HipException("DrawScreen: " + std::string(f) + " is not a full-screen kernel of this build");
    }
}

void HipCommandList::PrefilterEnv(DeviceTexture2DArray* sky, DeviceTexture2DArray* out) {
    if (!sky || !out) throw HipException("PrefilterEnv: null texture");
    mDispatchCount++;
    FlushPendingBloom();
    pbr_cube_f32 cube{(const float*)sky->DevicePtr(), sky->Size(), sky->MipLevels()};
    Check(pbr_prefilter_env(mCtx, &cube, out->Size(), out->MipLevels(), (pbr_half*)out->DevicePtr()), "pbr_prefilter_env");
    mPaddedEnv.erase(out);
}

void HipCommandList::Clustered(DeviceStructuredBuffer* clusters, DeviceStructuredBuffer* point_lights, int32 num_lights) {
    if (!clusters || !point_lights) throw HipException("Clustered: null buffer");
    mDispatchCount++;
    FlushPendingBloom();
    mNumLights = num_lights;
    Check(pbr_clustered(mCtx, &mGlobal, (const pbr_light*)point_lights->DevicePtr(), num_lights, (pbr_cluster*)clusters->DevicePtr()), "pbr_clustered");
}

void HipCommandList::Bloom(DeviceTexture2D* hdr, DeviceTexture2D* mip_chain, DeviceTexture2D* temp, float threshold, float knee) {
    if (!hdr || !mip_chain || !temp) throw HipException("Bloom: null texture");
    if (mip_chain->Width() != hdr->Width() || mip_chain->Height() != hdr->Height() || temp->Width() != hdr->Width() || temp->Height() != hdr->Height())
        throw HipException("Bloom: the mip chains must have the HDR target's size");
    mDispatchCount++;
    FlushPendingBloom();
    if (mTailOverlap == 2) BeginTail();
    mPendingBloom = PendingBloom{PendingBloom::Whole, hdr, mip_chain, temp, threshold, knee};
    if (!mFusedPasses) FlushPendingBloom();
}

void HipCommandList::FlushPendingBloom(uint32_t* hist, float min_log, float inv_range) {
    const PendingBloom p = mPendingBloom;
    mPendingBloom = PendingBloom{};
    if (p.What == PendingBloom::Whole) {
        pbr_half *hdr = (pbr_half*)p.Hdr->DevicePtr(), *a = (pbr_half*)p.MipChain->DevicePtr(), *b = (pbr_half*)p.Temp->DevicePtr();
        const uint32 w = p.Hdr->Width(), h = p.Hdr->Height();
        if (hist) {
            const Rect r = mInterior.w ? mInterior : Rect{0, 0, w, h};
            const uint32_t rect[4] = {r.x, r.y, r.w, r.h};
            Check(pbr_bloom_histogram(mCtx, hdr, w, h, w, a, b, p.Threshold, p.Knee, rect, min_log, inv_range, hist), "pbr_bloom_histogram");
        } else {
            Check(pbr_bloom(mCtx, hdr, w, h, w, a, b, p.Threshold, p.Knee), "pbr_bloom");
        }
    } else if (p.What == PendingBloom::Tiled) {
        IssueBloomTiled(p.Hdr, p.MipChain, p.Temp, hist, min_log, inv_range);
    }
}

void HipCommandList::IssueBloomTiled(DeviceTexture2D* hdr, DeviceTexture2D* mip_chain, DeviceTexture2D* temp, uint32_t* hist, float min_log, float inv_range) {
    const PixelRect s = mLayout.ShadedInBloom(), i = mLayout.InteriorInBloom();
    const uint32_t hdr_rect[4] = {s.x, s.y, s.w, s.h}, merge_rect[4] = {i.x, i.y, i.w, i.h};
    Check(pbr_bloom_tiled(mCtx, (pbr_half*)hdr->DevicePtr(), hdr->Width(), hdr_rect, mLayout.Bloom.w, mLayout.Bloom.h, (pbr_half*)mip_chain->DevicePtr(),
                          (pbr_half*)temp->DevicePtr(), merge_rect, min_log, inv_range, hist), "pbr_bloom_tiled");
}

void HipCommandList::HaloExchange(DeviceTexture2D* mip_chain) {
    if (mHaloPlan.empty()) return;
    pbr_half* level1 = (pbr_half*)mip_chain->MipPtr(1);
    const uint32 pitch = mLayout.Bloom.w / 2, rows = mLayout.Bloom.h / 2;
    const uint32_t n = (uint32_t)mHaloPlan.size();
    void* st = mHaloStaging->DevicePtr();
    const size_t bytes = mHaloStaging->Bytes();
    if (mHaloTransport == HaloTransport::Rccl) {
        Check(pbr_halo_exchange(mCtx, level1, pitch, rows, mHaloPlan.data(), n, st, bytes), "pbr_halo_exchange");
    } else {
        Check(pbr_halo_pack(mCtx, level1, pitch, rows, mHaloPlan.data(), n, st, bytes, 0), "pbr_halo_pack");
        Check(pbr_halo_pack(mCtx, level1, pitch, rows, mHaloPlan.data(), n, st, bytes, 1), "pbr_halo_pack(unpack)");
    }
}

void HipCommandList::BloomHalo(DeviceTexture2D* hdr, DeviceTexture2D* mip_chain, DeviceTexture2D* temp, float threshold, float knee) {
    if (!hdr || !mip_chain || !temp) throw HipException("BloomHalo: null texture");
    if (!mLayout.Halo) throw HipException("BloomHalo: the command list has no halo layout (SetLayout)");
    const TileLayout& l = mLayout;
    if (hdr->Width() != l.Shaded.w || hdr->Height() != l.Shaded.h) throw HipException("BloomHalo: the HDR target must cover the shaded rectangle");
    if (mip_chain->Width() != l.Bloom.w || mip_chain->Height() != l.Bloom.h || temp->Width() != l.Bloom.w || temp->Height() != l.Bloom.h)
        throw HipException("BloomHalo: the mip chains must cover the extended rectangle");
    mDispatchCount++;
    FlushPendingBloom();
    const PixelRect s = l.ShadedInBloom(), i = l.InteriorInShaded();
    const uint32_t rect[4] = {i.x / 2, i.y / 2, i.w / 2, i.h / 2};
    Check(pbr_bloom_prefilter_rect(mCtx, (pbr_half*)hdr->DevicePtr(), hdr->Width(), hdr->Height(), hdr->Width(), (pbr_half*)mip_chain->MipPtr(1),
                                   l.Bloom.w / 2, s.x / 2, s.y / 2, rect, threshold, knee), "pbr_bloom_prefilter_rect");
    HaloExchange(mip_chain);
    mPendingBloom = PendingBloom{PendingBloom::Tiled, hdr, mip_chain, temp, threshold, knee};
    if (!mFusedPasses) FlushPendingBloom();
}

void HipCommandList::DrawMesh(ShadingState* s) {
    if (!s || s->IsCompute()) throw HipException("DrawMesh: graphics shading state expected");
    const std::string_view f = s->File();
    mDispatchCount++;
    FlushPendingBloom();
    if (f != "skybox.hlsl") throw HipException("DrawMesh: " + std::string(f) + " is a raster shader without a kernel in this build");
    if (!mRenderTarget || !mDepthStencil) throw HipException("DrawMesh: render target / depth-stencil not bound (FrameGraph::PreparePass)");
    auto* sky = dynamic_cast<DeviceTexture2DArray*>(s->Texture("SkyBox").Texture);
    if (!sky) throw HipException("skybox: SkyBox is not bound to a cube texture");
    const uint32 w = mRenderTarget->Width(), h = mRenderTarget->Height();
    pbr_tile tile = mTile.w ? mTile : pbr_tile{0, 0, w, h, w, h};
    pbr_cube_f32 cube{(const float*)sky->DevicePtr(), sky->Size(), sky->MipLevels()};
// ... 40 lines not shown
```

direct12pbrrenderer_amd/host/HipCommandList.h:

```cpp
#pragma once
#include <string>
#include <vector>

#include "IPipeline.h"
#include "TileLayout.h"

namespace MRendererHip {

class HipCommandList {
public:
    explicit HipCommandList(int hip_device);
    ~HipCommandList();
    HipCommandList(const HipCommandList&) = delete;
    HipCommandList& operator=(const HipCommandList&) = delete;

    void BeginFrame() { mDispatchCount = 0; mEventLog.clear(); }
    void EndFrame();
    void SetFramesInFlight(uint32 k);
    void SetTailOverlap(int mode);
    int TailOverlap() const { return mTailOverlap; }
    uint32 FramesInFlight() const { return (uint32)mFrameFence.size() ? (uint32)mFrameFence.size() : 1; }
    void WaitIdle();

    void SetGlobalConstant(const ConstantBufferGlobal& g) { mGlobal = g; }
// ... 2 lines not shown
    void SetStencilRef(uint32 ref) { mStencilRef = ref; }
    void SetRenderTarget(DeviceTexture2D* rt) { mRenderTarget = rt; }
    void SetDepthStencil(DeviceTexture2D* ds) { mDepthStencil = ds; }
    void SetTile(const pbr_tile& tile) { mTile = tile; }
    void SetLayout(const TileLayout& layout);
    const TileLayout& Layout() const { return mLayout; }
    enum class HaloTransport { Rccl, Loopback };
    void SetHaloTransport(HaloTransport t) { mHaloTransport = t; }
    const std::vector<pbr_halo_peer>& HaloPlan() const { return mHaloPlan; }
    DeviceStructuredBuffer* HaloStaging() const { return mHaloStaging.get(); }
    bool HaloStripOffset(int rank, bool recv, size_t* offset, size_t* bytes) const;
    using Rect = PixelRect;
    void SetInterior(const Rect& r) { mInterior = r; }
    const Rect& Interior() const { return mInterior; }
    void SetExternalHistogram(const uint32* counts256);
    void CaptureHistogram(bool on) { mCaptureHistogram = on; }
    const std::vector<uint32>& CapturedHistogram() const { return mCapturedHistogram; }

    void Dispatch(ShadingState* state, uint32 thread_group_count_x, uint32 thread_group_count_y, uint32 thread_group_count_z);
    void DrawScreen(ShadingState* state);
    void DrawMesh(ShadingState* state);
    void EncodeGBuffer(ShadingState* state, const float* m0, const float* m1, const float* m2,
                       DeviceTexture2D* a, DeviceTexture2D* b, DeviceTexture2D* c);
    void RasterGBuffer(ShadingState* state, const pbr_vertex* vertices, uint32 n_vertices, const uint32_t* indices, uint32 n_indices,
                       const pbr_draw* draws, uint32 n_draws, uint32 max_triangles, DeviceTexture2D* a, DeviceTexture2D* b,
                       DeviceTexture2D* c, DeviceTexture2D* depth_stencil, void* scratch, size_t scratch_bytes,
                       const pbr_draw_maps* maps = nullptr, const pbr_texture2d* textures = nullptr, uint32 n_textures = 0);
    void Present(DeviceTexture2D* tex) { mPresented = tex; }

    void SetFusedPasses(bool on) { mFusedPasses = on; }
    bool FusedPasses() const { return mFusedPasses; }
    void PrefilterEnv(DeviceTexture2DArray* sky, DeviceTexture2DArray* out);
    void Clustered(DeviceStructuredBuffer* clusters, DeviceStructuredBuffer* point_lights, int32 num_lights);
    void Bloom(DeviceTexture2D* hdr, DeviceTexture2D* mip_chain, DeviceTexture2D* temp, float threshold, float knee);
    void BloomHalo(DeviceTexture2D* hdr, DeviceTexture2D* mip_chain, DeviceTexture2D* temp, float threshold, float knee);

    void BeginEvent(const char* name);
    void EndEvent();
    const std::vector<std::string>& EventLog() const { return mEventLog; }

    pbr_ctx* Context() const { return mCtx; }
    uint32 DispatchCount() const { return mDispatchCount; }
    DeviceTexture2D* Presented() const { return mPresented; }
    int32 NumLights() const { return mNumLights; }

private:
    void Check(pbr_status st, const char* what);
    void HaloExchange(DeviceTexture2D* mip_chain);
    struct PendingBloom {
        enum Kind { None, Whole, Tiled } What = None;
        DeviceTexture2D *Hdr = nullptr, *MipChain = nullptr, *Temp = nullptr;
        float Threshold = 0, Knee = 0;
    };
    void FlushPendingBloom(uint32_t* hist = nullptr, float min_log = 0.0f, float inv_range = 0.0f);
    void IssueBloomTiled(DeviceTexture2D* hdr, DeviceTexture2D* mip_chain, DeviceTexture2D* temp, uint32_t* hist, float min_log, float inv_range);

    pbr_ctx* mCtx = nullptr;
    ConstantBufferGlobal mGlobal{};
    uint32 mStencilRef = 0;
    uint32 mDispatchCount = 0;
    int32 mNumLights = 0;
    DeviceTexture2D* mPresented = nullptr;
    DeviceTexture2D* mRenderTarget = nullptr;
    DeviceTexture2D* mDepthStencil = nullptr;
    bool mFusedPasses = false;
    pbr_tile mTile{};
    Rect mInterior{};
    TileLayout mLayout{};
    HaloTransport mHaloTransport = HaloTransport::Rccl;
    std::vector<pbr_halo_peer> mHaloPlan;
    std::unique_ptr<DeviceStructuredBuffer> mHaloStaging;
    PendingBloom mPendingBloom;
    std::vector<hipEvent_t> mFrameFence;
    uint64_t mFrameIndex = 0;
    int mTailOverlap = 0;
    bool mInTail = false;
    void BeginTail();
    void EndTail();
    std::vector<uint32> mExternalHistogram, mCapturedHistogram;
    bool mCaptureHistogram = false;
    std::vector<std::string> mEventLog;
    std::map<const DeviceTexture2DArray*, std::unique_ptr<DeviceStructuredBuffer>> mPaddedEnv;
    std::map<const DeviceTexture2D*, std::unique_ptr<DeviceStructuredBuffer>> mFoldedLut;
};

class PixScope {
public:
    PixScope(HipCommandList* cmd, const char* name) : mCmd(cmd) { mCmd->BeginEvent(name); }
    ~PixScope() { mCmd->EndEvent(); }
    PixScope(const PixScope&) = delete;
    PixScope& operator=(const PixScope&) = delete;
private:
    HipCommandList* mCmd;
};
#define PBR_PIX_CAT2(a, b) a##b
#define PBR_PIX_CAT(a, b) PBR_PIX_CAT2(a, b)
#define PIXScope(cmd, name) ::MRendererHip::PixScope PBR_PIX_CAT(pix_scope_, __LINE__)((cmd), (name))

}
```

direct12pbrrenderer_amd/pipeline.py:

```python
import ctypes as C
from dataclasses import dataclass

import numpy as np
import torch

from .api import PbrContext
from .structs import (DRAW_MAPS_DTYPE, ENV_MIPS, HISTOGRAM_BINS, MAX_VIEWS, NO_MAP, GBuffer, Global, Tile, View)

DEFAULT_APRON = 256
HALO_SHADE_APRON = 4


@dataclass
class TileSpec:
    x0: int
    y0: int
    w: int
    h: int
    full_w: int
    full_h: int
    apron: int = 0
    shade_apron: int = None

    @property
    def ex0(self):
        return max(self.x0 - self.apron, 0)

    @property
    def ey0(self):
        return max(self.y0 - self.apron, 0)

    @property
    def ex1(self):
        return min(self.x0 + self.w + self.apron, self.full_w)

    @property
    def ey1(self):
        return min(self.y0 + self.h + self.apron, self.full_h)

    @property
    def ew(self):
        return self.ex1 - self.ex0

    @property
    def eh(self):
        return self.ey1 - self.ey0

    @property
    def ix(self):
        return self.x0 - self.ex0

    @property
    def iy(self):
        return self.y0 - self.ey0

    @property
    def halo(self):
        return self.shade_apron is not None and self.apron > 0

    @property
    def _sa(self):
        return self.shade_apron if self.halo else self.apron

    @property
    def sx0(self):
        return max(self.x0 - self._sa, 0)

    @property
    def sy0(self):
        return max(self.y0 - self._sa, 0)

    @property
    def sx1(self):
        return min(self.x0 + self.w + self._sa, self.full_w)

    @property
    def sy1(self):
        return min(self.y0 + self.h + self._sa, self.full_h)

    @property
    def sw(self):
        return self.sx1 - self.sx0

    @property
    def sh(self):
        return self.sy1 - self.sy0

    @property
    def six(self):
        return self.x0 - self.sx0
# ... 68 lines not shown

class HaloTransport:

    def __init__(self, kind, dist=None):
        assert kind in ("capi", "torch", "host")
        self.kind, self.dist = kind, dist

    def begin(self, fr):
        assert self.kind == "torch"
        if not fr.halo_n:
            return
        main = torch.cuda.current_stream(fr.ctx.torch_device)
        if getattr(self, "side", None) is None:
            self.side = torch.cuda.Stream(fr.ctx.torch_device)
        self.side.wait_stream(main)
        with torch.cuda.stream(self.side):
            fr.ctx.bind_torch_stream()
            self.exchange(fr)
        fr.ctx.bind_torch_stream()

    def end(self, fr):
        if fr.halo_n:
            torch.cuda.current_stream(fr.ctx.torch_device).wait_stream(self.side)

    def exchange(self, fr):
        ctx, a1, pitch, rows = fr.ctx, fr.level1, fr.spec.ew // 2, fr.spec.eh // 2
        if not fr.halo_n:
            return
        if self.kind == "capi":
            ctx.halo_exchange(a1, pitch, rows, fr.halo_peers, fr.halo_n, fr.halo_staging)
            return
        dist = self.dist
        ctx.halo_pack(a1, pitch, rows, fr.halo_peers, fr.halo_n, fr.halo_staging, unpack=False)
        ops, off, host = [], 0, self.kind == "host"
        st = fr.halo_staging
        if host:
            ctx.sync()
            st = st.cpu()
        for peer, send, _ in fr.halo_plan_local:
            if send:
                n = send[2] * send[3]
                ops.append(dist.P2POp(dist.isend, st[off:off + n], peer))
                off += n
        for peer, _, recv in fr.halo_plan_local:
            if recv:
                n = recv[2] * recv[3]
                ops.append(dist.P2POp(dist.irecv, st[off:off + n], peer))
                off += n
        for w in dist.batch_isend_irecv(ops):
            w.wait()
        if host:
            fr.halo_staging.copy_(st)
        ctx.halo_pack(a1, pitch, rows, fr.halo_peers, fr.halo_n, fr.halo_staging, unpack=True)


class DeferredFrame:

    def __init__(self, ctx: PbrContext, spec: TileSpec, g: Global, lights_np, lut, lut_res, env, env_size,
                 env_mips=ENV_MIPS, allreduce=None, sky=None, all_specs=None, rank=0, halo_transport=None, overlap=False, fused_exposure=False):
        self.ctx, self.spec, self.g = ctx, spec, g
        self.sky = sky
        self.n_lights = int(len(lights_np))
        self.lights = ctx.upload(lights_np) if self.n_lights else None
        self.lut, self.lut_res, self.env_size, self.env_mips = lut, lut_res, env_size, env_mips
        self.env = ctx.env_pad(env, env_size, env_mips)
        self.lut_fold = None
        self.refold_lut()
        self.allreduce = allreduce
        ew, eh = spec.ew, spec.eh
        self.clusters = ctx.alloc_clusters()
        self.hdr = ctx.zeros((spec.sh, spec.sw, 4), torch.float16)
        self.chain_a = ctx.alloc_bloom_chain(ew, eh)
        self.chain_b = ctx.alloc_bloom_chain(ew, eh)
        self.hist = ctx.zeros((HISTOGRAM_BINS,), torch.int32)
        self._tail_overlap = False
        self.avg = ctx.zeros((1,), torch.float32)
        self.fused_exposure = fused_exposure
        self._hist_next = ctx.zeros((HISTOGRAM_BINS,), torch.int32)
        self._avg_next = ctx.zeros((1,), torch.float32)
        self.ldr = ctx.zeros((spec.h, spec.w), torch.int32)
        self.gb = None
        self.mesh = None
        self.tile = Tile(spec.sx0, spec.sy0, spec.sw, spec.sh, spec.full_w, spec.full_h)
        self.halo_transport = halo_transport
        if spec.halo:
            assert all_specs is not None and halo_transport is not None, "halo mode needs every rank's TileSpec and a transport"
            from .structs import bloom_level_offset
            o = bloom_level_offset(ew, eh, 1)
            self.level1 = self.chain_a[o:o + (ew // 2) * (eh // 2)]
            hx, hy = spec.ex0 // 2, spec.ey0 // 2

            def loc(r):
                return None if r is None else (r[0] - hx, r[1] - hy, r[2] - r[0], r[3] - r[1])
            self.halo_plan_local = [(n, loc(snd), loc(rcv)) for n, snd, rcv in halo_plan(rank, len(all_specs), all_specs)]
            self.halo_peers, self.halo_n = ctx.halo_peers(self.halo_plan_local)
            self.halo_staging = ctx.zeros((max(ctx.halo_staging_bytes(self.halo_peers, self.halo_n) // 8, 1), 4), torch.float16)
        self.split = self._ring_core_split() if (spec.halo and overlap) else None

    def _ring_core_split(self):
        s = self.spec
        L, R = s.x0 > 0, s.x0 + s.w < s.full_w
        T, B = s.y0 > 0, s.y0 + s.h < s.full_h
        reach = s.apron + 4
        left = s.six + reach if L else 0
        right = (s.sw - s.six - s.w) + reach if R else 0
        top = s.siy + reach if T else 0
        bot = (s.sh - s.siy - s.h) + reach if B else 0
        mid_w, mid_h = s.sw - left - right, s.sh - top - bot
        if mid_w < 256 or mid_h < 64:
            return None
        ring = [r for r in ((0, 0, s.sw, top), (0, s.sh - bot, s.sw, bot), (0, top, left, mid_h), (s.sw - right, top, right, mid_h))
                if r[2] > 0 and r[3] > 0]
        core = (left, top, mid_w, mid_h)
        hb = s.apron // 2
        ox, oy, iw, ih = s.six // 2, s.siy // 2, s.w // 2, s.h // 2
        l, r_, t, b = (hb if L else 0), (hb if R else 0), (hb if T else 0), (hb if B else 0)
        l1_ring = [q for q in ((ox, oy, iw, t), (ox, oy + ih - b, iw, b), (ox, oy + t, l, ih - t - b), (ox + iw - r_, oy + t, r_, ih - t - b))
                   if q[2] > 0 and q[3] > 0]
        l1_core = (ox + l, oy + t, iw - l - r_, ih - t - b)
        return ring, core, l1_ring, l1_core

    def upload_gbuffer(self, gb_np):
        assert gb_np["A"].shape == (self.spec.sh, self.spec.sw)
        self.gb = {k: self.ctx.upload(v) for k, v in gb_np.items()}
        self.mesh = None

    def set_meshes(self, vertices, indices, draws, maps=None, textures=None):
        s, ctx = self.spec, self.ctx
        draws = np.ascontiguousarray(draws)
        n_tris = int((draws["index_count"] // 3).sum())
        textured = maps is not None and bool((np.asarray(maps).view(np.uint32) != NO_MAP).any())
        self.mesh = {"vertices": ctx.upload(vertices), "n_vertices": len(vertices),
                     "indices": ctx.upload(np.ascontiguousarray(indices, dtype=np.uint32)), "n_indices": len(indices),
                     "draws": ctx.upload(draws), "n_draws": len(draws), "max_triangles": n_tris,
                     "scratch": (ctx.alloc_textured_raster_scratch if textured else ctx.alloc_raster_scratch)(s.sw, s.sh, n_tris)}
        if textured:
            self.mesh["maps"] = ctx.upload(np.ascontiguousarray(maps, dtype=DRAW_MAPS_DTYPE))
            pairs = list(textures or [])
            if not all(isinstance(t, tuple) and len(t) == 2 for t in pairs):
                raise ValueError("set_meshes: textures are (device tensor, Texture2D) pairs (PbrContext.upload_texture)")
            self.mesh["texture_tensors"] = [t[0] for t in pairs]
            self.mesh["textures"] = [t[1] for t in pairs]
        self.gb = {"A": ctx.zeros((s.sh, s.sw), torch.int32), "B": ctx.zeros((s.sh, s.sw), torch.int32),
                   "C": ctx.zeros((s.sh, s.sw), torch.int32), "depth": ctx.zeros((s.sh, s.sw), torch.float32),
                   "stencil": ctx.zeros((s.sh, s.sw), torch.uint8)}

    def rasterize(self):
        m, gb = self.mesh, self.gb
        args = (self.g, self.tile, m["vertices"], m["n_vertices"], m["indices"], m["n_indices"], m["draws"], m["n_draws"],
                m["max_triangles"], gb["A"], gb["B"], gb["C"], gb["depth"], gb["stencil"], self.spec.sw, m["scratch"])
        if "maps" in m:
            self.ctx.gbuffer_raster_textured(*args, m["maps"], m["textures"])
        else:
            self.ctx.gbuffer_raster(*args)

    def set_sky_file(self, data, recompute_sh=False):
        from . import host
        size, mips, offsets, sh = host.parse_cubemap_file(data)
        staged = self.ctx.upload(np.frombuffer(bytes(data), dtype=np.uint8).copy())
        cube = self.ctx.bc6h_decode_cube([staged.data_ptr() + o for o in offsets], size, mips)
        if recompute_sh:
            pack = self.ctx.sh9_project(cube, size, mips)
            self.ctx.sync()
            sh = pack.cpu().numpy()
        else:
            self.ctx.sync()
        C.memmove(C.addressof(self.g.SkyBoxSH), np.ascontiguousarray(sh, dtype=np.float32).ctypes.data, 112)
        self.sky = (cube, size, mips)
        return sh

    def set_prev_luminance(self, v):
        self.avg.fill_(float(v))

    def _hdr_interior_ptr(self):
        s = self.spec
        return self.hdr.data_ptr() + 8 * (s.siy * s.sw + s.six)

    def clustered(self):
        self.ctx.clustered(self.g, self.lights, self.n_lights, self.clusters)

    def skybox(self):
        s = self.spec
        cube, size, mips = self.sky
        self.ctx.skybox(self.g, self.tile, cube, size, mips, self.gb["stencil"], s.sw, self.hdr, s.sw)

    def refold_lut(self):
        self.lut_fold = self.ctx.lut_fold_x(self.lut, self.lut_res, out=self.lut_fold if self.lut_fold is not None and self.lut_fold.shape[0] == self.lut_res else None)
        self._lut_folded = (self.lut.data_ptr(), self.lut_res)

    def _shade(self, rects):
        s = self.spec
        if self._lut_folded == (self.lut.data_ptr(), self.lut_res):
            self.ctx.deferred_shade_folded(self.g, self.tile, self.gb, s.sw, self.lut_fold, self.lut_res, self.env, self.env_size,
                                           self.env_mips, self.clusters, self.lights, self.n_lights, self.hdr, s.sw, rects)
        elif rects is None:
            self.ctx.deferred_shade(self.g, self.tile, self.gb, s.sw, self.lut, self.lut_res, self.env, self.env_size,
                                    self.env_mips, self.clusters, self.lights, self.n_lights, self.hdr, s.sw)
        else:
            self.ctx.deferred_shade_rects(self.g, self.tile, self.gb, s.sw, self.lut, self.lut_res, self.env, self.env_size,
                                          self.env_mips, self.clusters, self.lights, self.n_lights, self.hdr, s.sw, rects)

    def shade(self):
        self._shade(None)

    def shade_rects(self, rects):
        self._shade(rects)

    def prefilter_l1_rects(self, rects):
        s = self.spec
        self.ctx.bloom_prefilter_rects(self.hdr, s.sw, s.sh, s.sw, self.level1, s.ew // 2, (s.sx0 - s.ex0) // 2, (s.sy0 - s.ey0) // 2, rects)

    def shade_and_bloom_overlapped(self, histogram=True):
        ring, core, l1_ring, l1_core = self.split
        ctx, tr = self.ctx, self.halo_transport
        if tr.kind == "torch":
            self.shade_rects(ring)
            self.prefilter_l1_rects(l1_ring)
            tr.begin(self)
            self.shade_rects([core])
            tr.end(self)
        else:
            ctx.side_begin()
            self.shade_rects(ring)
            self.prefilter_l1_rects(l1_ring)
            if tr.kind == "host":
                ctx.side_end()
                ctx.side_join()
                tr.exchange(self)
            else:
                tr.exchange(self)
                ctx.side_end()
            self.shade_rects([core])
            ctx.side_join()
        self.prefilter_l1_rects([l1_core])
        self.halo_pyramid(histogram)

    def bloom(self):
        s = self.spec
        if s.halo:
            self.bloom_halo(histogram=False)
        else:
            self.ctx.bloom(self.hdr, s.ew, s.eh, s.ew, self.chain_a, self.chain_b)

    def histogram(self):
        s = self.spec
        self.ctx.lum_histogram(self._hdr_interior_ptr(), s.w, s.h, s.sw, self.hist)

    def halo_prefilter(self):
        s = self.spec
        self.ctx.bloom_prefilter_rect(self.hdr, s.sw, s.sh, s.sw, self.level1, s.ew // 2, (s.sx0 - s.ex0) // 2, (s.sy0 - s.ey0) // 2,
                                      (s.six // 2, s.siy // 2, s.w // 2, s.h // 2))

    def halo_exchange(self):
        self.halo_transport.exchange(self)

    def halo_pyramid(self, histogram=True):
        s = self.spec
        self.ctx.bloom_tiled(self.hdr, s.sw, (s.sx0 - s.ex0, s.sy0 - s.ey0, s.sw, s.sh), s.ew, s.eh, self.chain_a, self.chain_b,
                             (s.ix, s.iy, s.w, s.h), self.hist if histogram else None)

    def bloom_halo(self, histogram=True):
        self.halo_prefilter()
        self.halo_exchange()
        self.halo_pyramid(histogram)

    def bloom_histogram(self):
        s = self.spec
        if s.halo:
            self.bloom_halo(histogram=True)
        else:
            self.ctx.bloom_histogram(self.hdr, s.ew, s.eh, s.ew, self.chain_a, self.chain_b, (s.ix, s.iy, s.w, s.h), self.hist)

    def average(self):
        s = self.spec
        self.ctx.lum_average(self.hist, s.full_w * s.full_h, float(self.g.DeltaTime), self.avg)
# ... 203 lines not shown
```

direct12pbrrenderer_amd/structs.py:

```python
import ctypes as C

import numpy as np

CLUSTER_X, CLUSTER_Y, CLUSTER_Z = 24, 16, 8
MAX_LIGHTS_PER_CLUSTER = 32
MAX_SCENE_LIGHTS = 1024
NUM_CLUSTERS = CLUSTER_X * CLUSTER_Y * CLUSTER_Z
HISTOGRAM_BINS = 256
ENV_MIPS = 5
BLOOM_MIPS = 5
MIN_LOG_LUMINANCE = -10.0
MAX_LOG_LUMINANCE = 2.0
LOG_LUMINANCE_RANGE = MAX_LOG_LUMINANCE - MIN_LOG_LUMINANCE
INV_LOG_LUMINANCE_RANGE = float(np.float32(1.0) / np.float32(LOG_LUMINANCE_RANGE))
BLOOM_THRESHOLD = 1.0
BLOOM_KNEE = 0.5


class ShPack(C.Structure):
    _fields_ = [(n, C.c_float * 4) for n in ("sha_r", "shb_r", "sha_g", "shb_g", "sha_b", "shb_b", "shc")]


class Global(C.Structure):
    _fields_ = [
        ("SkyBoxSH", ShPack),
        ("InvView", C.c_float * 16),
        ("View", C.c_float * 16),
        ("Projection", C.c_float * 16),
        ("InvProjection", C.c_float * 16),
        ("CameraPos", C.c_float * 3),
        ("Ratio", C.c_float),
        ("Resolution", C.c_float * 2),
        ("Near", C.c_float),
        ("Far", C.c_float),
        ("Fov", C.c_float),
        ("DeltaTime", C.c_float),
        ("Time", C.c_float),
    ]


assert C.sizeof(Global) == 412


class Tile(C.Structure):
    _fields_ = [(n, C.c_uint32) for n in ("x0", "y0", "w", "h", "full_w", "full_h")]


class GBuffer(C.Structure):
    _fields_ = [
        ("A", C.c_void_p),
        ("B", C.c_void_p),
        ("C", C.c_void_p),
        ("depth", C.c_void_p),
        ("stencil", C.c_void_p),
        ("pitch", C.c_uint32),
    ]


MAX_VIEWS = 16


class View(C.Structure):
    _fields_ = [
        ("g", Global),
        ("gb", GBuffer),
        ("lights", C.c_void_p),
        ("num_lights", C.c_int32),
        ("clusters", C.c_void_p),
        ("hdr", C.c_void_p),
        ("hdr_pitch", C.c_uint32),
        ("chain_a", C.c_void_p),
        ("chain_b", C.c_void_p),
        ("hist256", C.c_void_p),
        ("avg", C.c_void_p),
        ("rgba8", C.c_void_p),
        ("out_pitch", C.c_uint32),
    ]


class HaloPeer(C.Structure):
    _fields_ = [("rank", C.c_int32), ("send", C.c_uint32 * 4), ("recv", C.c_uint32 * 4)]


class Vertex(C.Structure):
    _fields_ = [("position", C.c_float * 3), ("normal", C.c_float * 3), ("tangent", C.c_float * 3), ("color", C.c_float * 3),
                ("uv", C.c_float * 2)]


class Draw(C.Structure):
    _fields_ = [("Model", C.c_float * 16), ("InvModel", C.c_float * 16), ("Albedo", C.c_float * 3), ("Emission", C.c_float),
                ("Roughness", C.c_float), ("Metallic", C.c_float), ("first_index", C.c_uint32), ("index_count", C.c_uint32),
                ("base_vertex", C.c_int32)]


assert C.sizeof(Vertex) == 56 and C.sizeof(Draw) == 164
VERTEX_DTYPE = np.dtype([("position", np.float32, 3), ("normal", np.float32, 3), ("tangent", np.float32, 3),
                         ("color", np.float32, 3), ("uv", np.float32, 2)])
DRAW_DTYPE = np.dtype([("Model", np.float32, 16), ("InvModel", np.float32, 16), ("Albedo", np.float32, 3), ("Emission", np.float32),
                       ("Roughness", np.float32), ("Metallic", np.float32), ("first_index", np.uint32), ("index_count", np.uint32),
                       ("base_vertex", np.int32)])
assert VERTEX_DTYPE.itemsize == 56 and DRAW_DTYPE.itemsize == 164
RASTER_MAX_DRAWS = 65536
RASTER_MAX_TRIANGLES = 1 << 22
RASTER_MAX_SIZE = 8192


class Texture2D(C.Structure):
    _fields_ = [("texels", C.c_void_p), ("width", C.c_uint32), ("height", C.c_uint32), ("mip_levels", C.c_uint32),
                ("format", C.c_uint32)]


assert C.sizeof(Texture2D) == 24
DRAW_MAPS_DTYPE = np.dtype([("albedo", np.uint32), ("normal", np.uint32), ("roughness", np.uint32), ("metallic", np.uint32),
                            ("ao", np.uint32)])
assert DRAW_MAPS_DTYPE.itemsize == 20
MAP_NAMES = DRAW_MAPS_DTYPE.names
NO_MAP = 0xFFFFFFFF
RASTER_MAX_TEXTURES = 64
TEX_MAX_SIZE = 16384
TEX_R8G8B8A8_UNORM, TEX_B8G8R8A8_UNORM, TEX_B8G8R8A8_UNORM_SRGB, TEX_R8_UNORM = 28, 87, 91, 61
TEX_FORMATS = {TEX_R8G8B8A8_UNORM: (4, False), TEX_B8G8R8A8_UNORM: (4, False), TEX_B8G8R8A8_UNORM_SRGB: (4, True),
               TEX_R8_UNORM: (1, False)}
TEX_BC1_BLOCKS = 0x100


def texture2d_bytes(width, height, mip_levels, fmt):
    width, height, mip_levels, fmt = int(width), int(height), int(mip_levels), int(fmt)
    if fmt & ~(0xFF | TEX_BC1_BLOCKS) or (fmt & 0xFF) not in TEX_FORMATS:
# ... 58 lines not shown
```

include/pbr_hip.h:

```cpp
#ifndef PBR_HIP_H
#define PBR_HIP_H

#include <stdint.h>
#include <stddef.h>

#ifdef __cplusplus
extern "C" {
#endif

typedef int pbr_status;
enum {
    PBR_OK              =  0,
    PBR_ERR_INVALID     = -1,
    PBR_ERR_HIP         = -2,
    PBR_ERR_NOMEM       = -3,
    PBR_ERR_UNSUPPORTED = -4,
    PBR_ERR_COMM        = -5
};

typedef struct pbr_ctx pbr_ctx;
typedef uint16_t pbr_half;

#define PBR_CLUSTER_X              24
#define PBR_CLUSTER_Y              16
// ... 57 lines not shown

typedef struct pbr_cube_f32 {
    const float* data;
    uint32_t size;
    uint32_t mips;
} pbr_cube_f32;

size_t pbr_cube_texels(uint32_t size, uint32_t mips);
size_t pbr_cube_mip_offset(uint32_t size, uint32_t mip);
size_t pbr_env_padded_texels(uint32_t size, uint32_t mips);
size_t pbr_env_padded_mip_offset(uint32_t size, uint32_t mip);
size_t pbr_bloom_chain_texels(uint32_t w, uint32_t h);
size_t pbr_bloom_level_offset(uint32_t w, uint32_t h, uint32_t level);

pbr_status  pbr_ctx_create(int hip_device, pbr_ctx** out);
void        pbr_ctx_destroy(pbr_ctx* ctx);
pbr_status  pbr_ctx_set_stream(pbr_ctx* ctx, void* hip_stream);
pbr_status  pbr_ctx_use_own_stream(pbr_ctx* ctx);
void*       pbr_ctx_get_stream(const pbr_ctx* ctx);
pbr_status  pbr_ctx_side_begin(pbr_ctx* ctx);
pbr_status  pbr_ctx_side_end(pbr_ctx* ctx);
pbr_status  pbr_ctx_side_join(pbr_ctx* ctx);
pbr_status  pbr_ctx_set_bloom_shader_order(pbr_ctx* ctx, int on);
const char* pbr_last_error(const pbr_ctx* ctx);
pbr_status  pbr_sync(pbr_ctx* ctx);
const char* pbr_version(void);
const char* pbr_runtime_error(void);
int pbr_runtime_mismatch_dirs(const char* hip_dir, const char* torch_dir);

pbr_status pbr_brdf_lut(pbr_ctx* ctx, uint32_t res, pbr_half* out_rg);

pbr_status pbr_rgbe_decode(pbr_ctx* ctx, const uint8_t* rgbe, size_t texels, float* out_rgba);

pbr_status pbr_cube_gen_mips(pbr_ctx* ctx, float* cube_data, uint32_t size, uint32_t mips);

#define PBR_BC6H_MAX_SIZE 8192u
size_t pbr_bc6h_chain_bytes(uint32_t size, uint32_t mip_levels);
pbr_status pbr_bc6h_decode_cube(pbr_ctx* ctx, const void* const face_blocks[6], uint32_t size, uint32_t mip_levels, float* out_rgba);

pbr_status pbr_prefilter_env(pbr_ctx* ctx, const pbr_cube_f32* sky, uint32_t size, uint32_t mips,
                             pbr_half* out_rgba);
pbr_status pbr_prefilter_env_mip(pbr_ctx* ctx, const pbr_cube_f32* sky, uint32_t size, uint32_t mip_level,
                                 float roughness, pbr_half* out_mip_rgba);

pbr_status pbr_env_pad(pbr_ctx* ctx, const pbr_half* env_rgba, uint32_t size, uint32_t mips, pbr_half* out_padded);

pbr_status pbr_sh9_project(pbr_ctx* ctx, const pbr_cube_f32* sky, float* out_pack);

pbr_status pbr_cluster_build(pbr_ctx* ctx, const pbr_global* g, pbr_cluster* clusters);

pbr_status pbr_cluster_cull(pbr_ctx* ctx, const pbr_global* g, const pbr_light* lights, int n,
                            pbr_cluster* clusters);
pbr_status pbr_clustered(pbr_ctx* ctx, const pbr_global* g, const pbr_light* lights, int num_lights,
                         pbr_cluster* clusters);

pbr_status pbr_deferred_shade(pbr_ctx* ctx, const pbr_global* g, const pbr_tile* tile,
                              const pbr_gbuffer* gb,
                              const pbr_half* lut, uint32_t lut_res,
                              const pbr_half* env_padded, uint32_t env_size, uint32_t env_mips,
                              const pbr_cluster* clusters, const pbr_light* lights, int num_lights,
                              pbr_half* hdr, uint32_t hdr_pitch);

pbr_status pbr_deferred_shade_rects(pbr_ctx* ctx, const pbr_global* g, const pbr_tile* tile,
                                    const pbr_gbuffer* gb,
                                    const pbr_half* lut, uint32_t lut_res,
                                    const pbr_half* env_padded, uint32_t env_size, uint32_t env_mips,
                                    const pbr_cluster* clusters, const pbr_light* lights, int num_lights,
                                    pbr_half* hdr, uint32_t hdr_pitch, const uint32_t (*rects)[4], uint32_t n_rects);

pbr_status pbr_lut_fold_x(pbr_ctx* ctx, const pbr_half* lut, uint32_t lut_res, float* out_fold);

pbr_status pbr_deferred_shade_folded(pbr_ctx* ctx, const pbr_global* g, const pbr_tile* tile,
                                     const pbr_gbuffer* gb,
                                     const float* lut_fold, uint32_t lut_res,
                                     const pbr_half* env_padded, uint32_t env_size, uint32_t env_mips,
                                     const pbr_cluster* clusters, const pbr_light* lights, int num_lights,
                                     pbr_half* hdr, uint32_t hdr_pitch);
pbr_status pbr_deferred_shade_rects_folded(pbr_ctx* ctx, const pbr_global* g, const pbr_tile* tile,
                                           const pbr_gbuffer* gb,
                                           const float* lut_fold, uint32_t lut_res,
                                           const pbr_half* env_padded, uint32_t env_size, uint32_t env_mips,
                                           const pbr_cluster* clusters, const pbr_light* lights, int num_lights,
                                           pbr_half* hdr, uint32_t hdr_pitch, const uint32_t (*rects)[4], uint32_t n_rects);

pbr_status pbr_deferred_shade_f32(pbr_ctx* ctx, const pbr_global* g, const pbr_tile* tile,
                                  const pbr_gbuffer* gb,
                                  const pbr_half* lut, uint32_t lut_res,
                                  const pbr_half* env_padded, uint32_t env_size, uint32_t env_mips,
                                  const pbr_cluster* clusters, const pbr_light* lights, int num_lights,
                                  float* hdr_f32, uint32_t hdr_pitch);

pbr_status pbr_skybox(pbr_ctx* ctx, const pbr_global* g, const pbr_tile* tile, const pbr_cube_f32* sky,
                      const uint8_t* stencil, uint32_t pitch, pbr_half* hdr, uint32_t hdr_pitch);

pbr_status pbr_gbuffer_encode(pbr_ctx* ctx, const float* m0, const float* m1, const float* m2,
                              uint32_t w, uint32_t h, uint32_t pitch, uint32_t* A, uint32_t* B, uint32_t* C);

typedef struct pbr_vertex {
    float position[3];
    float normal[3];
    float tangent[3];
    float color[3];
    float uv[2];
} pbr_vertex;
typedef struct pbr_draw {
    float Model[16];
    float InvModel[16];
    float Albedo[3];
    float Emission;
    float Roughness;
    float Metallic;
    uint32_t first_index;
    uint32_t index_count;
    int32_t  base_vertex;
} pbr_draw;
#define PBR_RASTER_MAX_DRAWS     65536u
#define PBR_RASTER_MAX_TRIANGLES (1u << 22)
#define PBR_RASTER_MAX_SIZE      8192u
size_t pbr_gbuffer_raster_scratch_bytes(uint32_t w, uint32_t h, uint32_t n_triangles);
size_t pbr_gbuffer_raster_min_scratch_bytes(uint32_t w, uint32_t h, uint32_t n_triangles);
pbr_status pbr_gbuffer_raster(pbr_ctx* ctx, const pbr_global* g, const pbr_tile* tile,
                              const pbr_vertex* vertices, uint32_t n_vertices, const uint32_t* indices, uint32_t n_indices,
                              const pbr_draw* draws, uint32_t n_draws, uint32_t max_triangles,
                              uint32_t* A, uint32_t* B, uint32_t* C, float* depth, uint8_t* stencil, uint32_t pitch,
                              void* scratch, size_t scratch_bytes);

#define PBR_TEX_R8G8B8A8_UNORM       28u
#define PBR_TEX_B8G8R8A8_UNORM       87u
#define PBR_TEX_B8G8R8A8_UNORM_SRGB  91u
#define PBR_TEX_R8_UNORM             61u
#define PBR_TEX_MAX_SIZE             16384u
#define PBR_TEX_BC1_BLOCKS           0x100u
typedef struct pbr_texture2d {
    const void* texels;
    uint32_t width, height;
    uint32_t mip_levels;
    uint32_t format;
} pbr_texture2d;
size_t pbr_texture2d_bytes(uint32_t width, uint32_t height, uint32_t mip_levels, uint32_t format);
pbr_status pbr_bc1_decode(pbr_ctx* ctx, const void* blocks, uint32_t width, uint32_t height, uint32_t mip_levels,
                          uint32_t stored_format, void* out);
pbr_status pbr_texture2d_gen_mips(pbr_ctx* ctx, void* texels, uint32_t width, uint32_t height, uint32_t mip_levels, uint32_t format);
pbr_status pbr_bc1_encode(pbr_ctx* ctx, const void* texels, uint32_t width, uint32_t height, uint32_t mip_levels,
                          uint32_t stored_format, void* blocks_out);
#define PBR_NO_MAP                   0xffffffffu
#define PBR_RASTER_MAX_TEXTURES      64u
typedef struct pbr_draw_maps {
    uint32_t albedo, normal, roughness, metallic, ao;
} pbr_draw_maps;
size_t pbr_gbuffer_raster_textured_scratch_bytes(uint32_t w, uint32_t h, uint32_t n_triangles);
size_t pbr_gbuffer_raster_textured_min_scratch_bytes(uint32_t w, uint32_t h, uint32_t n_triangles);
pbr_status pbr_gbuffer_raster_textured(pbr_ctx* ctx, const pbr_global* g, const pbr_tile* tile,
                                       const pbr_vertex* vertices, uint32_t n_vertices, const uint32_t* indices, uint32_t n_indices,
                                       const pbr_draw* draws, uint32_t n_draws, uint32_t max_triangles,
                                       uint32_t* A, uint32_t* B, uint32_t* C, float* depth, uint8_t* stencil, uint32_t pitch,
                                       void* scratch, size_t scratch_bytes,
                                       const pbr_draw_maps* maps, const pbr_texture2d* textures, uint32_t n_textures);

pbr_status pbr_bloom_prefilter(pbr_ctx* ctx, const pbr_half* hdr, uint32_t w, uint32_t h,
                               uint32_t pitch, pbr_half* out, float threshold, float knee);
pbr_status pbr_blur_h(pbr_ctx* ctx, const pbr_half* in, uint32_t iw, uint32_t ih,
                      pbr_half* out, uint32_t ow, uint32_t oh);
pbr_status pbr_blur_v(pbr_ctx* ctx, const pbr_half* in, uint32_t iw, uint32_t ih,
                      pbr_half* out, uint32_t ow, uint32_t oh);
pbr_status pbr_bloom_upsample_add(pbr_ctx* ctx, const pbr_half* upper, uint32_t uw, uint32_t uh,
                                  const pbr_half* lower, uint32_t lw, uint32_t lh, pbr_half* out);
// ... 84 lines not shown
```

Before: 18470.

## Prebuild shading tables in cluster cull and stream them into the shade kernel

```diff
diff --git a/direct12pbrrenderer_amd/_lib.py b/direct12pbrrenderer_amd/_lib.py
--- a/direct12pbrrenderer_amd/_lib.py
+++ b/direct12pbrrenderer_amd/_lib.py
@@ -1,7 +1,7 @@
 import ctypes as C
 import os
 
-from .structs import CubeF32, GBuffer, Global, HaloPeer, Texture2D, Tile, View
+from .structs import CubeF32, GBuffer, Global, HaloPeer, ShadeTables, Texture2D, Tile, View
 
 _HERE = os.path.dirname(os.path.abspath(__file__))
 LIB_PATH = os.environ.get("PBR_HIP_LIB", os.path.join(_HERE, "libpbr_hip.so"))
@@ -47,6 +47,13 @@
                                          _vp, _u32, _vp, _u32, _u32, _vp, _vp, _int, _vp, _u32]),
     "pbr_deferred_shade_rects_folded": (_int, [_vp, C.POINTER(Global), C.POINTER(Tile), C.POINTER(GBuffer),
                                                _vp, _u32, _vp, _u32, _u32, _vp, _vp, _int, _vp, _u32, _vp, _u32]),
+    "pbr_shade_tables_bytes": (_sz, [_u32, _u32]),
+    "pbr_clustered_tables": (_int, [_vp, C.POINTER(Global), _vp, _int, _vp, C.POINTER(ShadeTables)]),
+    "pbr_shade_geometry_tables": (_int, [_vp, C.POINTER(Tile), C.POINTER(ShadeTables)]),
+    "pbr_deferred_shade_tabled": (_int, [_vp, C.POINTER(Global), C.POINTER(Tile), C.POINTER(GBuffer),
+                                         _vp, _u32, _vp, _u32, _u32, _vp, _vp, _int, _vp, _u32, C.POINTER(ShadeTables)]),
+    "pbr_deferred_shade_rects_tabled": (_int, [_vp, C.POINTER(Global), C.POINTER(Tile), C.POINTER(GBuffer),
+                                               _vp, _u32, _vp, _u32, _u32, _vp, _vp, _int, _vp, _u32, _vp, _u32, C.POINTER(ShadeTables)]),
     "pbr_skybox": (_int, [_vp, C.POINTER(Global), C.POINTER(Tile), C.POINTER(CubeF32), _vp, _u32, _vp, _u32]),
     "pbr_gbuffer_encode": (_int, [_vp, _vp, _vp, _vp, _u32, _u32, _u32, _vp, _vp, _vp]),
     "pbr_gbuffer_raster_scratch_bytes": (_sz, [_u32, _u32, _u32]),
diff --git a/direct12pbrrenderer_amd/api.py b/direct12pbrrenderer_amd/api.py
--- a/direct12pbrrenderer_amd/api.py
+++ b/direct12pbrrenderer_amd/api.py
@@ -4,7 +4,7 @@
 import torch
 
 from . import _lib
-from .structs import (Texture2D, BLOOM_KNEE, BLOOM_THRESHOLD, CLUSTER_DTYPE, ENV_MIPS, HISTOGRAM_BINS,
+from .structs import (ShadeTables, Texture2D, BLOOM_KNEE, BLOOM_THRESHOLD, CLUSTER_DTYPE, ENV_MIPS, HISTOGRAM_BINS,
                       INV_LOG_LUMINANCE_RANGE, LIGHT_DTYPE, LOG_LUMINANCE_RANGE, MIN_LOG_LUMINANCE,
                       NUM_CLUSTERS, DRAW_DTYPE, DRAW_MAPS_DTYPE, TEX_BC1_BLOCKS, TEX_FORMATS, VERTEX_DTYPE, CubeF32, GBuffer, Global, HaloPeer, Tile, View, bloom_chain_texels, bc6h_chain_bytes, cube_texels, env_padded_texels, texture2d_bytes)
 
@@ -221,6 +221,29 @@
             arr = self._rects(rects)
             self._check(self.lib.pbr_deferred_shade_rects_folded(*head, C.cast(arr, C.c_void_p), len(rects)))
 
+    def alloc_shade_tables(self, w, h):
+        n = int(self.lib.pbr_shade_tables_bytes(int(w), int(h)))
+        buf = self.zeros((n // 4,), torch.int32)
+        return buf, ShadeTables(buf.data_ptr(), n, 0, 0, 0, Tile(0, 0, 0, 0, 0, 0))
+
+    def clustered_tables(self, g: Global, lights, n, clusters, tables: ShadeTables):
+        self._check(self.lib.pbr_clustered_tables(self.h, C.byref(g), _ptr(lights), int(n), _ptr(clusters), C.byref(tables)))
+
+    def shade_geometry_tables(self, tile: Tile, tables: ShadeTables):
+        self._check(self.lib.pbr_shade_geometry_tables(self.h, C.byref(tile), C.byref(tables)))
+
+    def deferred_shade_tabled(self, g: Global, tile: Tile, gb, pitch, lut_fold, lut_res, env, env_size, env_mips,
+                              clusters, lights, num_lights, hdr, hdr_pitch, tables: ShadeTables, rects=None):
+        s = GBuffer(gb["A"].data_ptr(), gb["B"].data_ptr(), gb["C"].data_ptr(), gb["depth"].data_ptr(),
+                    gb["stencil"].data_ptr(), pitch)
+        head = (self.h, C.byref(g), C.byref(tile), C.byref(s), _ptr(lut_fold), lut_res, _ptr(env), env_size, env_mips,
+                _ptr(clusters), _ptr(lights), int(num_lights), _ptr(hdr), hdr_pitch)
+        if rects is None:
+            self._check(self.lib.pbr_deferred_shade_tabled(*head, C.byref(tables)))
+        else:
+            arr = self._rects(rects)
+            self._check(self.lib.pbr_deferred_shade_rects_tabled(*head, C.cast(arr, C.c_void_p), len(rects), C.byref(tables)))
+
     def deferred_shade_f32(self, g: Global, tile: Tile, gb, pitch, lut, lut_res, env, env_size, env_mips,
                            clusters, lights, num_lights, hdr_f32, hdr_pitch):
         s = GBuffer(gb["A"].data_ptr(), gb["B"].data_ptr(), gb["C"].data_ptr(), gb["depth"].data_ptr(),
diff --git a/direct12pbrrenderer_amd/csrc/cluster.hip b/direct12pbrrenderer_amd/csrc/cluster.hip
--- a/direct12pbrrenderer_amd/csrc/cluster.hip
+++ b/direct12pbrrenderer_amd/csrc/cluster.hip
@@ -63,6 +63,42 @@
 struct ClusterViews { ClusterView v[PBR_MAX_VIEWS]; };
 static_assert(sizeof(ClusterViews) <= 4096 - 256, "k_cluster_cull<.., ClusterViews>: kernel arguments over 4 KiB");
 
+template <bool BUILD, bool TABLES>
+__device__ __forceinline__ void cull_cluster(const ClusterParams& p, const pbr_light* __restrict__ lights, int n, pbr_cluster* __restrict__ clusters,
+                                             int ci, int lane, uint32_t* __restrict__ staged) {
+    pbr_cluster* c = clusters + ci;
+    float mn[3], mx[3];
+    int count = 0;
+    if (BUILD) {
+        cluster_bounds(p, ci, mn, mx);
+        if (lane < 3) { c->MinBound[lane] = mn[lane]; c->MaxBound[lane] = mx[lane]; }
+    } else {
+        mn[0] = c->MinBound[0]; mn[1] = c->MinBound[1]; mn[2] = c->MinBound[2];
+        mx[0] = c->MaxBound[0]; mx[1] = c->MaxBound[1]; mx[2] = c->MaxBound[2];
+        count = c->NumLights;
+        count = min(max(count, 0), PBR_MAX_LIGHTS_PER_CLUSTER);
+    }
+    for (int base = 0; base < n && count < PBR_MAX_LIGHTS_PER_CLUSTER; base += 64) {
+        const int i = base + lane;
+        bool hit = false;
+        if (i < n) hit = light_hits(p, lights[i], mn, mx);
+        const unsigned long long mask = __ballot(hit);
+        const int pos = count + __popcll(mask & ((1ull << lane) - 1ull));
+        if (hit && pos < PBR_MAX_LIGHTS_PER_CLUSTER) {
+            c->LightIndex[pos] = i;
+            if (TABLES) staged[2 + pos] = 4u * (uint32_t)i;
+        }
+        count = min(count + __popcll(mask), PBR_MAX_LIGHTS_PER_CLUSTER);
+    }
+    if (lane == 0) c->NumLights = count;
+    if (TABLES) {
+        static_assert(PBR_MAX_LIGHTS_PER_CLUSTER == STAGED_LIST_DWORDS - 2, "staged list: one entry per list slot");
+        if (lane >= count && lane < PBR_MAX_LIGHTS_PER_CLUSTER) staged[2 + lane] = 4u * (uint32_t)n;
+        if (lane == 32) staged[0] = (uint32_t)staged_list_padded(count);
+        if (lane == 33) staged[1] = 0u;
+    }
+}
+
 template <bool BUILD, class VS = NoViews>
 __global__ __launch_bounds__(256) void k_cluster_cull(ClusterParams p_, const pbr_light* __restrict__ lights_, int n_, VS vs,
                                                         pbr_cluster* __restrict__ clusters_) {
@@ -76,28 +112,39 @@
     const int lane = threadIdx.x & 63;
     const int ci = blockIdx.x * 4 + (threadIdx.x >> 6);
     if (ci >= PBR_NUM_CLUSTERS) return;
-    pbr_cluster* c = clusters + ci;
-    float mn[3], mx[3];
-    int count = 0;
-    if (BUILD) {
-        cluster_bounds(p, ci, mn, mx);
-        if (lane < 3) { c->MinBound[lane] = mn[lane]; c->MaxBound[lane] = mx[lane]; }
-    } else {
-        mn[0] = c->MinBound[0]; mn[1] = c->MinBound[1]; mn[2] = c->MinBound[2];
-        mx[0] = c->MaxBound[0]; mx[1] = c->MaxBound[1]; mx[2] = c->MaxBound[2];
-        count = c->NumLights;
-        count = min(max(count, 0), PBR_MAX_LIGHTS_PER_CLUSTER);
-    }
-    for (int base = 0; base < n && count < PBR_MAX_LIGHTS_PER_CLUSTER; base += 64) {
-        const int i = base + lane;
-        bool hit = false;
-        if (i < n) hit = light_hits(p, lights[i], mn, mx);
-        const unsigned long long mask = __ballot(hit);
-        const int pos = count + __popcll(mask & ((1ull << lane) - 1ull));
-        if (hit && pos < PBR_MAX_LIGHTS_PER_CLUSTER) c->LightIndex[pos] = i;
-        count = min(count + __popcll(mask), PBR_MAX_LIGHTS_PER_CLUSTER);
-    }
-    if (lane == 0) c->NumLights = count;
+    cull_cluster<BUILD, false>(p, lights, n, clusters, ci, lane, nullptr);
+}
+
+__global__ __launch_bounds__(256) void k_cluster_cull_tables(ClusterParams p, const pbr_light* __restrict__ lights, int n,
+                                                               pbr_cluster* __restrict__ clusters, uint32_t* __restrict__ tables) {
+    if (blockIdx.x < PBR_NUM_CLUSTERS / 4) {
+        const int ci = blockIdx.x * 4 + (threadIdx.x >> 6);
+        cull_cluster<true, true>(p, lights, n, clusters, ci, threadIdx.x & 63, tables + PBR_TABLES_LISTS + ci * STAGED_LIST_DWORDS);
+        return;
+    }
+    const int stride = shade_light_stride(n);
+    float* planes = reinterpret_cast<float*>(tables + PBR_TABLES_PLANES);
+    int my_safe = 1, my_same = 1;
+    const float att0 = n > 0 ? lights[0].C0 : 1.0f, att1 = n > 0 ? lights[0].C1 : 0.0f, att2 = n > 0 ? lights[0].C2 : 0.0f;
+    for (int i = threadIdx.x; i < stride; i += 256) {
+        float v[9] = {0.0f, 0.0f, 0.0f, 0.0f, 0.0f, 0.0f, 0.0f, 0.0f, 0.0f};
+        if (i < n) {
+            const pbr_light l = lights[i];
+            my_safe &= (l.C0 >= EPSILON_F) & (l.C1 >= 0.0f) & (l.C2 >= 0.0f);
+            my_same &= (l.C0 == att0) & (l.C1 == att1) & (l.C2 == att2);
+            v[0] = l.Position[0]; v[1] = l.Position[1]; v[2] = l.Position[2];
+            v[3] = l.Color[0] * l.Intensity; v[4] = l.Color[1] * l.Intensity; v[5] = l.Color[2] * l.Intensity;
+            v[6] = l.C0; v[7] = l.C1; v[8] = l.C2;
+        } else if (i == n) {
+            v[0] = v[1] = v[2] = 1.0e15f;
+            v[6] = 1.0f;
+        }
+#pragma unroll
+        for (int k = 0; k < 9; k++) planes[k * stride + i] = v[k];
+    }
+    for (uint32_t d = 9u * (uint32_t)stride + threadIdx.x; d < PBR_TABLES_LISTS - PBR_TABLES_PLANES; d += 256u) planes[d] = 0.0f;
+    const int q_safe = (__syncthreads_and(my_safe) != 0 ? 1 : 0) | (__syncthreads_and(my_same) != 0 ? 2 : 0);
+    if (threadIdx.x < 4) tables[PBR_TABLES_HEADER + threadIdx.x] = threadIdx.x == 0 ? (uint32_t)q_safe : threadIdx.x == 1 ? (uint32_t)n : threadIdx.x == 2 ? (uint32_t)stride : 0u;
 }
 
 static ClusterParams make_params(const pbr_global* g) {
@@ -139,6 +186,21 @@
     PBR_CHECK(ctx, "pbr_clustered", cull_args_bad(g, true, lights, n));
     hipLaunchKernelGGL(k_cluster_cull<true>, dim3(PBR_NUM_CLUSTERS / 4), dim3(256), 0, ctx->stream, make_params(g), lights, n, NoViews{}, clusters);
     return launched(ctx, "k_cluster_cull<build>");
+}
+
+size_t pbr_shade_tables_bytes(uint32_t w, uint32_t h) { return ((size_t)PBR_TABLES_GEOM + 2u * (size_t)w + 2u * (size_t)h) * 4u; }
+
+pbr_status pbr_clustered_tables(pbr_ctx* ctx, const pbr_global* g, const pbr_light* lights, int n, pbr_cluster* clusters, pbr_shade_tables* tables) {
+    if (!ctx) return PBR_ERR_INVALID;
+    PBR_REQUIRE(ctx, g && clusters && tables, "pbr_clustered_tables: null pointer");
+    PBR_CHECK(ctx, "pbr_clustered_tables", cull_args_bad(g, true, lights, n));
+    PBR_REQUIRE(ctx, tables->dev && ((uintptr_t)tables->dev & 15u) == 0 && tables->bytes >= (uint64_t)PBR_TABLES_GEOM * 4u,
+                "pbr_clustered_tables: the tables buffer must be 16-byte aligned and hold pbr_shade_tables_bytes()");
+    tables->built &= ~PBR_TABLES_BUILT_FRAME;
+    hipLaunchKernelGGL(k_cluster_cull_tables, dim3(PBR_NUM_CLUSTERS / 4 + 1), dim3(256), 0, ctx->stream, make_params(g), lights, n, clusters, (uint32_t*)tables->dev);
+    const pbr_status r = launched(ctx, "k_cluster_cull_tables");
+    if (r == PBR_OK) { tables->built |= PBR_TABLES_BUILT_FRAME; tables->num_lights = n; tables->list_pad = 2u * SHADE_WALK_TRIPS; }
+    return r;
 }
 
 pbr_status pbr_clustered_views(pbr_ctx* ctx, const pbr_view* views, uint32_t n) {
diff --git a/direct12pbrrenderer_amd/csrc/pbr_device.hpp b/direct12pbrrenderer_amd/csrc/pbr_device.hpp
--- a/direct12pbrrenderer_amd/csrc/pbr_device.hpp
+++ b/direct12pbrrenderer_amd/csrc/pbr_device.hpp
@@ -11,6 +11,16 @@
 constexpr float TWO_PI_F = (float)(2.0 * 3.14159265359);
 
 typedef _Float16 h16;
+
+#ifndef SHADE_WALK_TRIPS
+#define SHADE_WALK_TRIPS 2
+#endif
+constexpr int STAGED_LIST_DWORDS = 34;
+__host__ __device__ inline int staged_list_padded(int cnt) {
+    const int up = (cnt + 2 * SHADE_WALK_TRIPS - 1) & ~(2 * SHADE_WALK_TRIPS - 1);
+    return up > 2 * SHADE_WALK_TRIPS ? up : 2 * SHADE_WALK_TRIPS;
+}
+__host__ __device__ inline int shade_light_stride(int n_lights) { return n_lights <= 256 ? 257 : PBR_MAX_SCENE_LIGHTS + 1; }
 
 struct V3 { float x, y, z; };
 __device__ __forceinline__ V3 v3(float x, float y, float z) { return V3{x, y, z}; }
diff --git a/direct12pbrrenderer_amd/csrc/shade.hip b/direct12pbrrenderer_amd/csrc/shade.hip
--- a/direct12pbrrenderer_amd/csrc/shade.hip
+++ b/direct12pbrrenderer_amd/csrc/shade.hip
@@ -97,9 +97,6 @@
 constexpr int SHADE_ROWS = 8;
 constexpr int MAX_STAGED_TILES = 12;
 constexpr int LIST_STRIDE = 34;
-#ifndef SHADE_WALK_TRIPS
-#define SHADE_WALK_TRIPS 2
-#endif
 constexpr int WALK_TRIPS = SHADE_WALK_TRIPS;
 static_assert(WALK_TRIPS == 2 || WALK_TRIPS == 4, "a staging thread converts four entries: the padded length must be a multiple of four that divides 32");
 
@@ -557,6 +554,99 @@
 #endif
 }
 
+__global__ __launch_bounds__(256) void k_shade_geometry_tables(uint32_t x0, uint32_t y0, uint32_t w, uint32_t h, uint32_t full_w, uint32_t full_h, float2* __restrict__ geom) {
+    const uint32_t t = blockIdx.x * 256u + threadIdx.x;
+    if (t < w) {
+        const float u = ((float)(x0 + t) + 0.5f) / (float)full_w;
+        const float ndc_x = 2.0f * u - 1.0f;
+        const int sx = clampi((int)floorf(u * (float)PBR_CLUSTER_X), 0, PBR_CLUSTER_X - 1);
+        geom[t] = make_float2(ndc_x * 0.5f, __int_as_float(sx));
+    } else if (t < w + h) {
+        const float v = ((float)(y0 + (t - w)) + 0.5f) / (float)full_h;
+        const float ndc_y = 1.0f - 2.0f * v;
+        const int sy = clampi((int)floorf((1.0f - v) * (float)PBR_CLUSTER_Y), 0, PBR_CLUSTER_Y - 1);
+        geom[t] = make_float2(ndc_y * 0.5f, __int_as_float(sy));
+    }
+}
+
+template <int LSTRIDE>
+__global__ __launch_bounds__(SHADE_BLOCK, SHADE_MIN_WAVES) void k_deferred_shade_tabled(ShadeParams p, int n_lights, int max_clusters, ShadeRects rc, const uint32_t* __restrict__ tab) {
+    extern __shared__ float4 lds_raw[];
+    __shared__ uint32_t s_mip_off[16];
+    __shared__ float4 s_row[SHADE_ROWS];
+    const unsigned long long t_start = SHADE_NOW();
+    (void)t_start;
+    if (threadIdx.x < 16) s_mip_off[threadIdx.x] = p.env_mip_off[threadIdx.x];
+    float* llds = reinterpret_cast<float*>(lds_raw);
+    uint32_t* lists = reinterpret_cast<uint32_t*>(llds + ((LIGHT_PLANES * LSTRIDE + 1) & ~1));
+    {
+        constexpr int N4 = (LIGHT_PLANES * LSTRIDE) / 4, TAIL = (LIGHT_PLANES * LSTRIDE) & 3;
+        const uint4* src = reinterpret_cast<const uint4*>(tab + PBR_TABLES_PLANES);
+#pragma unroll 1
+        for (int i = threadIdx.x; i < N4; i += SHADE_BLOCK) reinterpret_cast<uint4*>(llds)[i] = src[i];
+        if (threadIdx.x < (uint32_t)TAIL) llds[4 * N4 + threadIdx.x] = __uint_as_float(tab[PBR_TABLES_PLANES + 4 * N4 + threadIdx.x]);
+    }
+    uint32_t r = 0;
+    while (r + 1 < rc.n && blockIdx.x >= rc.first[r + 1]) r++;
+    const uint32_t lb = blockIdx.x - rc.first[r];
+    const uint32_t bx0 = rc.x0[r] + (lb % rc.cols[r]) * SHADE_BLOCK, x_end = rc.x0[r] + rc.w[r];
+    const uint32_t by = lb / rc.cols[r], nb_big = rc.nb_big[r], rows_big = rc.rows_big, rows_small = rc.rows_small;
+    const uint32_t y_begin = rc.y0[r] + (by < nb_big ? by * rows_big : nb_big * rows_big + (by - nb_big) * rows_small);
+    const uint32_t y_end = min(y_begin + (by < nb_big ? rows_big : rows_small), rc.y0[r] + rc.h[r]);
+    const uint32_t lds_base = (uint32_t)(uintptr_t)(lds_cf*)llds;
+    const uint2* cols = reinterpret_cast<const uint2*>(tab + PBR_TABLES_GEOM);
+    const uint2* rows = cols + p.w;
+    const uint32_t bx1 = min(bx0 + SHADE_BLOCK, x_end) - 1;
+    const int tile_x0 = (int)cols[bx0].y, tile_x1 = (int)cols[bx1].y;
+    const int ty_a = (int)rows[y_begin].y, ty_b = (int)rows[y_end - 1].y;
+    const int tile_y0 = min(ty_a, ty_b), tile_y1 = max(ty_a, ty_b);
+    const int tiles_x = tile_x1 - tile_x0 + 1;
+    {
+        static_assert(LIST_STRIDE == STAGED_LIST_DWORDS && PBR_CLUSTER_Z * LIST_STRIDE % 4 == 0, "staged run");
+        const int run4 = tiles_x * (PBR_CLUSTER_Z * LIST_STRIDE / 4);
+        const int cap4 = max_clusters * LIST_STRIDE / 4;
+#pragma unroll 1
+        for (int j = 0; j <= tile_y1 - tile_y0; j++) {
+            const uint4* src = reinterpret_cast<const uint4*>(tab + PBR_TABLES_LISTS + ((tile_y0 + j) * PBR_CLUSTER_X + tile_x0) * (PBR_CLUSTER_Z * LIST_STRIDE));
+            uint2* dst = reinterpret_cast<uint2*>(lists) + 2 * (j * run4);
+            const int n4 = min(run4, cap4 - j * run4);
+#pragma unroll 1
+            for (int q = threadIdx.x; q < n4; q += SHADE_BLOCK) {
+                const uint32_t m = (2u * (uint32_t)q) % 17u;
+                const uint32_t lo = m == 0u ? 0u : lds_base, hi = m == 16u ? 0u : lds_base;
+                const uint4 v = src[q];
+                dst[2 * q] = make_uint2(v.x + lo, v.y + lo);
+                dst[2 * q + 1] = make_uint2(v.z + hi, v.w + hi);
+            }
+        }
+    }
+    if (threadIdx.x < (uint32_t)SHADE_ROWS) {
+        const uint2 e = rows[min(y_begin + threadIdx.x, p.h - 1u)];
+        const float cvv_y = __uint_as_float(e.x) * p.near_height;
+        const uint32_t row_list = (uint32_t)(((int)e.y - tile_y0) * tiles_x * (PBR_CLUSTER_Z * LIST_STRIDE));
+        s_row[threadIdx.x] = make_float4(p.InvView[1] * cvv_y, p.InvView[4] * cvv_y, p.InvView[7] * cvv_y, __uint_as_float(row_list));
+    }
+    const int q_safe = (int)tab[PBR_TABLES_HEADER];
+    const uint32_t px = bx0 + threadIdx.x;
+    const uint2 ce = cols[min(px, p.w - 1u)];
+    const float cvv_x = __uint_as_float(ce.x) * p.near_width;
+    const uint32_t col_list = (uint32_t)(((int)ce.y - tile_x0) * (PBR_CLUSTER_Z * LIST_STRIDE));
+    __syncthreads();
+    SHADE_ISTAMP(blockIdx.x, 0, t_start);
+    SHADE_ISTAMP(blockIdx.x, 1, SHADE_NOW());
+    SHADE_ISTAMP(blockIdx.x, 3, ((unsigned long long)(y_end - y_begin) << 48) | blockIdx.x);
+#ifndef PBR_SHADE_TIMING
+    if (px >= x_end) return;
+    for (uint32_t py = y_begin; py < y_end; py++)
+        shade_pixel<true, LSTRIDE, false, true>(p, llds, lists, s_mip_off, n_lights, q_safe, px, py, s_row[py - y_begin], cvv_x, col_list);
+#else
+    if (px < x_end)
+        for (uint32_t py = y_begin; py < y_end; py++)
+            shade_pixel<true, LSTRIDE, false, true>(p, llds, lists, s_mip_off, n_lights, q_safe, px, py, s_row[py - y_begin], cvv_x, col_list);
+    SHADE_ISTAMP_MAX(blockIdx.x, 2, SHADE_NOW());
+#endif
+}
+
 extern "C" {
 
 pbr_status pbr_env_pad(pbr_ctx* ctx, const pbr_half* env, uint32_t size, uint32_t mips, pbr_half* out_padded) {
@@ -651,16 +741,24 @@
 }
 
 template <bool F32OUT, bool LUTFOLD, class VS>
-static pbr_status shade_dispatch(pbr_ctx* ctx, const ShadeParams& p, int num_lights, int max_lights, const ShadeRects& rc, uint32_t n_views, const VS& vs) {
+static pbr_status shade_dispatch(pbr_ctx* ctx, const ShadeParams& p, int num_lights, int max_lights, const ShadeRects& rc, uint32_t n_views, const VS& vs,
+                                 const uint32_t* tables = nullptr) {
     const uint32_t span_x = (uint32_t)((uint64_t)(SHADE_BLOCK - 1) * PBR_CLUSTER_X / p.full_w) + 2;
     const uint32_t span_y = (uint32_t)((uint64_t)(SHADE_ROWS - 1) * PBR_CLUSTER_Y / p.full_h) + 2;
-    const int lstride = max_lights <= 256 ? 257 : PBR_MAX_SCENE_LIGHTS + 1;
+    const int lstride = shade_light_stride(max_lights);
     const size_t plane_bytes = (size_t)((LIGHT_PLANES * lstride + 1) & ~1) * sizeof(float);
     const bool staged = span_x * span_y <= (uint32_t)MAX_STAGED_TILES &&
                         plane_bytes + (size_t)span_x * span_y * PBR_CLUSTER_Z * LIST_STRIDE * sizeof(uint32_t) <= 65536;
     const int max_clusters = staged ? (int)(span_x * span_y) * PBR_CLUSTER_Z : 0;
     const size_t lds = plane_bytes + (size_t)max_clusters * LIST_STRIDE * sizeof(uint32_t);
     const dim3 grid(rc.first[rc.n], n_views), blk(SHADE_BLOCK);
+    if constexpr (std::is_same_v<VS, NoViews> && LUTFOLD && !F32OUT) {
+        if (tables && staged) {
+            if (lstride == 257) hipLaunchKernelGGL((k_deferred_shade_tabled<257>), grid, blk, lds, ctx->stream, p, num_lights, max_clusters, rc, tables);
+            else hipLaunchKernelGGL((k_deferred_shade_tabled<PBR_MAX_SCENE_LIGHTS + 1>), grid, blk, lds, ctx->stream, p, num_lights, max_clusters, rc, tables);
+            return launched(ctx, "k_deferred_shade_tabled");
+        }
+    }
     if (staged && lstride == 257) hipLaunchKernelGGL((k_deferred_shade<true, 257, F32OUT, VS, LUTFOLD>), grid, blk, lds, ctx->stream, p, num_lights, max_clusters, rc, vs);
     else if (staged) hipLaunchKernelGGL((k_deferred_shade<true, PBR_MAX_SCENE_LIGHTS + 1, F32OUT, VS, LUTFOLD>), grid, blk, lds, ctx->stream, p, num_lights, max_clusters, rc, vs);
     else if (lstride == 257) hipLaunchKernelGGL((k_deferred_shade<false, 257, F32OUT, VS, LUTFOLD>), grid, blk, lds, ctx->stream, p, num_lights, 0, rc, vs);
@@ -674,7 +772,7 @@
                                const pbr_half* env, uint32_t env_size, uint32_t env_mips,
                                const pbr_cluster* clusters, const pbr_light* lights, int num_lights,
                                pbr_half* hdr, float* hdr_f32, uint32_t hdr_pitch,
-                               const uint32_t (*rects)[4] = nullptr, uint32_t n_rects = 0) {
+                               const uint32_t (*rects)[4] = nullptr, uint32_t n_rects = 0, const pbr_shade_tables* tables = nullptr, bool tabled = false) {
     if (!ctx) return PBR_ERR_INVALID;
     const char* who = "pbr_deferred_shade";
     PBR_REQUIRE(ctx, g && tile && gb, "pbr_deferred_shade: null pointer");
@@ -689,12 +787,20 @@
         const uint32_t* q = rects[r];
         PBR_REQUIRE(ctx, q[2] >= 1 && q[3] >= 1 && q[0] + q[2] <= tile->w && q[1] + q[3] <= tile->h, "pbr_deferred_shade: rectangle outside the tile");
     }
+    if (tabled) {
+        PBR_REQUIRE(ctx, tables && tables->dev, "pbr_deferred_shade_tabled: null tables");
+        PBR_REQUIRE(ctx, (tables->built & PBR_TABLES_BUILT_FRAME) && (tables->built & PBR_TABLES_BUILT_GEOMETRY), "pbr_deferred_shade_tabled: only one half of the tables is built");
+        PBR_REQUIRE(ctx, tables->num_lights == num_lights, "pbr_deferred_shade_tabled: the tables were built for another light count");
+        PBR_REQUIRE(ctx, memcmp(&tables->tile, tile, sizeof(pbr_tile)) == 0, "pbr_deferred_shade_tabled: the tables were built for another tile");
+        PBR_REQUIRE(ctx, tables->list_pad == 2u * WALK_TRIPS, "pbr_deferred_shade_tabled: the cull padded the lists for another walk (SHADE_WALK_TRIPS differs between cluster.hip and shade.hip)");
+        PBR_REQUIRE(ctx, ((uintptr_t)tables->dev & 15u) == 0 && tables->bytes >= pbr_shade_tables_bytes(tile->w, tile->h), "pbr_deferred_shade_tabled: tables buffer misaligned or too small");
+    }
     ShadeParams p = shade_params(g, LUTFOLD ? nullptr : (const pbr_half*)lut, lut_res, env, env_size, env_mips);
     if (LUTFOLD) p.lut_fold = (const float*)lut;
     p.x0 = tile->x0; p.y0 = tile->y0; p.w = tile->w; p.h = tile->h; p.full_w = tile->full_w; p.full_h = tile->full_h;
     p.A = gb->A; p.B = gb->B; p.C = gb->C; p.depth = gb->depth; p.stencil = gb->stencil; p.pitch = gb->pitch;
     p.clusters = clusters; p.lights = lights; p.hdr = hdr; p.hdr_pitch = hdr_pitch; p.hdr_f32 = hdr_f32;
-    return shade_dispatch<F32OUT, LUTFOLD>(ctx, p, num_lights, num_lights, shade_schedule(ctx, rects, n_rects, 1), 1, NoViews{});
+    return shade_dispatch<F32OUT, LUTFOLD>(ctx, p, num_lights, num_lights, shade_schedule(ctx, rects, n_rects, 1), 1, NoViews{}, tabled ? (const uint32_t*)tables->dev : nullptr);
 }
 
 extern "C" {
@@ -740,6 +846,38 @@
                                            pbr_half* hdr, uint32_t hdr_pitch, const uint32_t (*rects)[4], uint32_t n_rects) {
     if (ctx && !rects) return pbr::fail(ctx, PBR_ERR_INVALID, "pbr_deferred_shade_rects_folded: null rectangle list");
     return shade_launch<false, true>(ctx, g, tile, gb, lut_fold, lut_res, env, env_size, env_mips, clusters, lights, num_lights, hdr, nullptr, hdr_pitch, rects, n_rects);
+}
+
+pbr_status pbr_shade_geometry_tables(pbr_ctx* ctx, const pbr_tile* tile, pbr_shade_tables* tables) {
+    if (!ctx) return PBR_ERR_INVALID;
+    PBR_REQUIRE(ctx, tile && tables, "pbr_shade_geometry_tables: null pointer");
+    PBR_REQUIRE(ctx, tile->w >= 1 && tile->h >= 1 && tile->w <= 65535 && tile->h <= 65535, "pbr_shade_geometry_tables: bad tile size");
+    PBR_REQUIRE(ctx, tile->x0 + tile->w <= tile->full_w && tile->y0 + tile->h <= tile->full_h, "pbr_shade_geometry_tables: tile outside frame");
+    PBR_REQUIRE(ctx, tables->dev && ((uintptr_t)tables->dev & 15u) == 0 && tables->bytes >= pbr_shade_tables_bytes(tile->w, tile->h),
+                "pbr_shade_geometry_tables: the tables buffer must be 16-byte aligned and hold pbr_shade_tables_bytes(w, h)");
+    tables->built &= ~PBR_TABLES_BUILT_GEOMETRY;
+    hipLaunchKernelGGL(k_shade_geometry_tables, dim3((tile->w + tile->h + 255) / 256), dim3(256), 0, ctx->stream, tile->x0, tile->y0, tile->w, tile->h,
+                       tile->full_w, tile->full_h, reinterpret_cast<float2*>((uint32_t*)tables->dev + PBR_TABLES_GEOM));
+    const pbr_status r = launched(ctx, "k_shade_geometry_tables");
+    if (r == PBR_OK) { tables->built |= PBR_TABLES_BUILT_GEOMETRY; tables->tile = *tile; }
+    return r;
+}
+
+pbr_status pbr_deferred_shade_tabled(pbr_ctx* ctx, const pbr_global* g, const pbr_tile* tile, const pbr_gbuffer* gb,
+                                     const float* lut_fold, uint32_t lut_res,
+                                     const pbr_half* env, uint32_t env_size, uint32_t env_mips,
+                                     const pbr_cluster* clusters, const pbr_light* lights, int num_lights,
+                                     pbr_half* hdr, uint32_t hdr_pitch, const pbr_shade_tables* tables) {
+    return shade_launch<false, true>(ctx, g, tile, gb, lut_fold, lut_res, env, env_size, env_mips, clusters, lights, num_lights, hdr, nullptr, hdr_pitch, nullptr, 0, tables, true);
+}
+
+pbr_status pbr_deferred_shade_rects_tabled(pbr_ctx* ctx, const pbr_global* g, const pbr_tile* tile, const pbr_gbuffer* gb,
+                                           const float* lut_fold, uint32_t lut_res,
+                                           const pbr_half* env, uint32_t env_size, uint32_t env_mips,
+                                           const pbr_cluster* clusters, const pbr_light* lights, int num_lights,
+                                           pbr_half* hdr, uint32_t hdr_pitch, const uint32_t (*rects)[4], uint32_t n_rects, const pbr_shade_tables* tables) {
+    if (ctx && !rects) return pbr::fail(ctx, PBR_ERR_INVALID, "pbr_deferred_shade_rects_tabled: null rectangle list");
+    return shade_launch<false, true>(ctx, g, tile, gb, lut_fold, lut_res, env, env_size, env_mips, clusters, lights, num_lights, hdr, nullptr, hdr_pitch, rects, n_rects, tables, true);
 }
 
 pbr_status pbr_deferred_shade_f32(pbr_ctx* ctx, const pbr_global* g, const pbr_tile* tile, const pbr_gbuffer* gb,
diff --git a/direct12pbrrenderer_amd/host/HipCommandList.cpp b/direct12pbrrenderer_amd/host/HipCommandList.cpp
--- a/direct12pbrrenderer_amd/host/HipCommandList.cpp
+++ b/direct12pbrrenderer_amd/host/HipCommandList.cpp
@@ -274,11 +274,13 @@
         mPaddedEnv.erase(out);
     } else if (f == "clustered_compute.hlsl") {
         ExpectGroups(f, gx, gy, gz, 1, 1, 1);
+        StaleShadeTables(s->Buffer("Clusters"));
         Check(pbr_cluster_build(mCtx, &mGlobal, (pbr_cluster*)s->Buffer("Clusters")->DevicePtr()), "pbr_cluster_build");
     } else if (f == "clustered_culling.hlsl") {
         ExpectGroups(f, gx, gy, gz, 1, 1, 1);
         const auto& c = s->Constants<ClusteredShaderConstant>();
         mNumLights = c.NumLight;
+        StaleShadeTables(s->Buffer("Clusters"));
         Check(pbr_cluster_cull(mCtx, &mGlobal, (const pbr_light*)s->Buffer("PointLights")->DevicePtr(), c.NumLight,
                                (pbr_cluster*)s->Buffer("Clusters")->DevicePtr()), "pbr_cluster_cull");
     } else if (f == "bloom_prefilter.hlsl") {
@@ -374,10 +376,22 @@
             Check(pbr_lut_fold_x(mCtx, (const pbr_half*)lut->DevicePtr(), lut->Width(), (float*)folded->DevicePtr()), "pbr_lut_fold_x");
         }
         if (mStencilRef != 0) throw HipException("deferred_shading: only stencil ref 0 is supported");
-        Check(pbr_deferred_shade_folded(mCtx, &mGlobal, &tile, &gb, (const float*)folded->DevicePtr(), lut->Width(),
-                                        (const pbr_half*)padded->DevicePtr(), env->Size(), env->MipLevels(),
-                                        (const pbr_cluster*)s->Buffer("Clusters")->DevicePtr(), (const pbr_light*)s->Buffer("PointLights")->DevicePtr(),
-                                        mNumLights, (pbr_half*)mRenderTarget->DevicePtr(), w), "pbr_deferred_shade_folded");
+        auto tables = mShadeTables.find(s->Buffer("Clusters"));
+        if (tables != mShadeTables.end() && (tables->second.desc.built & PBR_TABLES_BUILT_FRAME) && tables->second.desc.num_lights == mNumLights &&
+            tables->second.lights == s->Buffer("PointLights")) {
+            pbr_shade_tables& d = tables->second.desc;
+            if (!(d.built & PBR_TABLES_BUILT_GEOMETRY) || memcmp(&d.tile, &tile, sizeof(tile)) != 0)
+                Check(pbr_shade_geometry_tables(mCtx, &tile, &d), "pbr_shade_geometry_tables");
+            Check(pbr_deferred_shade_tabled(mCtx, &mGlobal, &tile, &gb, (const float*)folded->DevicePtr(), lut->Width(),
+                                            (const pbr_half*)padded->DevicePtr(), env->Size(), env->MipLevels(),
+                                            (const pbr_cluster*)s->Buffer("Clusters")->DevicePtr(), (const pbr_light*)s->Buffer("PointLights")->DevicePtr(),
+                                            mNumLights, (pbr_half*)mRenderTarget->DevicePtr(), w, &d), "pbr_deferred_shade_tabled");
+        } else {
+            Check(pbr_deferred_shade_folded(mCtx, &mGlobal, &tile, &gb, (const float*)folded->DevicePtr(), lut->Width(),
+                                            (const pbr_half*)padded->DevicePtr(), env->Size(), env->MipLevels(),
+                                            (const pbr_cluster*)s->Buffer("Clusters")->DevicePtr(), (const pbr_light*)s->Buffer("PointLights")->DevicePtr(),
+                                            mNumLights, (pbr_half*)mRenderTarget->DevicePtr(), w), "pbr_deferred_shade_folded");
+        }
     } else if (f == "hdr_tone_mapping.hlsl") {
         Mip in = MipOf(s->Texture("LuminanceTexture"));
         const Rect r = mInterior.w ? mInterior : Rect{0, 0, in.w, in.h};
@@ -404,7 +418,18 @@
     mDispatchCount++;
     FlushPendingBloom();
     mNumLights = num_lights;
-    Check(pbr_clustered(mCtx, &mGlobal, (const pbr_light*)point_lights->DevicePtr(), num_lights, (pbr_cluster*)clusters->DevicePtr()), "pbr_clustered");
+    ShadeTables& t = mShadeTables[clusters];
+    if (!t.buf) {
+        t.buf = std::make_unique<DeviceStructuredBuffer>((uint32)pbr_shade_tables_bytes(65535, 65535), 16);
+        t.desc = pbr_shade_tables{t.buf->DevicePtr(), pbr_shade_tables_bytes(65535, 65535), 0, 0, 0, {}};
+    }
+    t.lights = point_lights;
+    Check(pbr_clustered_tables(mCtx, &mGlobal, (const pbr_light*)point_lights->DevicePtr(), num_lights, (pbr_cluster*)clusters->DevicePtr(), &t.desc), "pbr_clustered_tables");
+}
+
+void HipCommandList::StaleShadeTables(const DeviceStructuredBuffer* clusters) {
+    auto t = mShadeTables.find(clusters);
+    if (t != mShadeTables.end()) t->second.desc.built &= ~PBR_TABLES_BUILT_FRAME;
 }
 
 void HipCommandList::Bloom(DeviceTexture2D* hdr, DeviceTexture2D* mip_chain, DeviceTexture2D* temp, float threshold, float knee) {
diff --git a/direct12pbrrenderer_amd/host/HipCommandList.h b/direct12pbrrenderer_amd/host/HipCommandList.h
--- a/direct12pbrrenderer_amd/host/HipCommandList.h
+++ b/direct12pbrrenderer_amd/host/HipCommandList.h
@@ -108,6 +108,13 @@
     std::vector<std::string> mEventLog;
     std::map<const DeviceTexture2DArray*, std::unique_ptr<DeviceStructuredBuffer>> mPaddedEnv;
     std::map<const DeviceTexture2D*, std::unique_ptr<DeviceStructuredBuffer>> mFoldedLut;
+    struct ShadeTables {
+        std::unique_ptr<DeviceStructuredBuffer> buf;
+        pbr_shade_tables desc{};
+        const DeviceStructuredBuffer* lights = nullptr;
+    };
+    std::map<const DeviceStructuredBuffer*, ShadeTables> mShadeTables;
+    void StaleShadeTables(const DeviceStructuredBuffer* clusters);
 };
 
 class PixScope {
diff --git a/direct12pbrrenderer_amd/pipeline.py b/direct12pbrrenderer_amd/pipeline.py
--- a/direct12pbrrenderer_amd/pipeline.py
+++ b/direct12pbrrenderer_amd/pipeline.py
@@ -5,7 +5,7 @@
 import torch
 
 from .api import PbrContext
-from .structs import (DRAW_MAPS_DTYPE, ENV_MIPS, HISTOGRAM_BINS, MAX_VIEWS, NO_MAP, GBuffer, Global, Tile, View)
+from .structs import (DRAW_MAPS_DTYPE, ENV_MIPS, HISTOGRAM_BINS, MAX_VIEWS, NO_MAP, TABLES_BUILT_FRAME, TABLES_BUILT_GEOMETRY, GBuffer, Global, Tile, View)
 
 DEFAULT_APRON = 256
 HALO_SHADE_APRON = 4
@@ -240,6 +240,9 @@
         self.gb = None
         self.mesh = None
         self.tile = Tile(spec.sx0, spec.sy0, spec.sw, spec.sh, spec.full_w, spec.full_h)
+        self.tabled = True
+        self.tables_buf, self.tables = ctx.alloc_shade_tables(spec.sw, spec.sh)
+        ctx.shade_geometry_tables(self.tile, self.tables)
         self.halo_transport = halo_transport
         if spec.halo:
             assert all_specs is not None and halo_transport is not None, "halo mode needs every rank's TileSpec and a transport"
@@ -335,7 +338,10 @@
         return self.hdr.data_ptr() + 8 * (s.siy * s.sw + s.six)
 
     def clustered(self):
-        self.ctx.clustered(self.g, self.lights, self.n_lights, self.clusters)
+        if self.tabled:
+            self.ctx.clustered_tables(self.g, self.lights, self.n_lights, self.clusters, self.tables)
+        else:
+            self.ctx.clustered(self.g, self.lights, self.n_lights, self.clusters)
 
     def skybox(self):
         s = self.spec
@@ -348,7 +354,11 @@
 
     def _shade(self, rects):
         s = self.spec
-        if self._lut_folded == (self.lut.data_ptr(), self.lut_res):
+        folded = self._lut_folded == (self.lut.data_ptr(), self.lut_res)
+        if folded and self.tabled and self.tables.built == TABLES_BUILT_FRAME | TABLES_BUILT_GEOMETRY and self.tables.num_lights == self.n_lights:
+            self.ctx.deferred_shade_tabled(self.g, self.tile, self.gb, s.sw, self.lut_fold, self.lut_res, self.env, self.env_size,
+                                           self.env_mips, self.clusters, self.lights, self.n_lights, self.hdr, s.sw, self.tables, rects)
+        elif folded:
             self.ctx.deferred_shade_folded(self.g, self.tile, self.gb, s.sw, self.lut_fold, self.lut_res, self.env, self.env_size,
                                            self.env_mips, self.clusters, self.lights, self.n_lights, self.hdr, s.sw, rects)
         elif rects is None:
diff --git a/direct12pbrrenderer_amd/structs.py b/direct12pbrrenderer_amd/structs.py
--- a/direct12pbrrenderer_amd/structs.py
+++ b/direct12pbrrenderer_amd/structs.py
@@ -44,6 +44,14 @@
 
 class Tile(C.Structure):
     _fields_ = [(n, C.c_uint32) for n in ("x0", "y0", "w", "h", "full_w", "full_h")]
+
+
+class ShadeTables(C.Structure):
+    _fields_ = [("dev", C.c_void_p), ("bytes", C.c_uint64), ("built", C.c_uint32), ("num_lights", C.c_int32), ("list_pad", C.c_uint32), ("tile", Tile)]
+
+
+TABLES_HEADER, TABLES_PLANES, TABLES_LISTS, TABLES_GEOM = 0, 4, 9232, 113680
+TABLES_BUILT_FRAME, TABLES_BUILT_GEOMETRY = 1, 2
 
 
 class GBuffer(C.Structure):
diff --git a/include/pbr_hip.h b/include/pbr_hip.h
--- a/include/pbr_hip.h
+++ b/include/pbr_hip.h
@@ -163,6 +163,41 @@
                                            const pbr_half* env_padded, uint32_t env_size, uint32_t env_mips,
                                            const pbr_cluster* clusters, const pbr_light* lights, int num_lights,
                                            pbr_half* hdr, uint32_t hdr_pitch, const uint32_t (*rects)[4], uint32_t n_rects);
+
+#define PBR_TABLES_HEADER 0u
+#define PBR_TABLES_PLANES 4u
+#define PBR_TABLES_LISTS  9232u
+#define PBR_TABLES_GEOM   113680u
+#define PBR_TABLES_BUILT_FRAME 1u
+#define PBR_TABLES_BUILT_GEOMETRY 2u
+typedef struct pbr_shade_tables {
+    void* dev;
+    uint64_t bytes;
+    uint32_t built;
+    int32_t num_lights;
+    uint32_t list_pad;
+    pbr_tile tile;
+} pbr_shade_tables;
+size_t pbr_shade_tables_bytes(uint32_t w, uint32_t h);
+
+pbr_status pbr_clustered_tables(pbr_ctx* ctx, const pbr_global* g, const pbr_light* lights, int num_lights,
+                                pbr_cluster* clusters, pbr_shade_tables* tables);
+
+pbr_status pbr_shade_geometry_tables(pbr_ctx* ctx, const pbr_tile* tile, pbr_shade_tables* tables);
+
+pbr_status pbr_deferred_shade_tabled(pbr_ctx* ctx, const pbr_global* g, const pbr_tile* tile,
+                                     const pbr_gbuffer* gb,
+                                     const float* lut_fold, uint32_t lut_res,
+                                     const pbr_half* env_padded, uint32_t env_size, uint32_t env_mips,
+                                     const pbr_cluster* clusters, const pbr_light* lights, int num_lights,
+                                     pbr_half* hdr, uint32_t hdr_pitch, const pbr_shade_tables* tables);
+pbr_status pbr_deferred_shade_rects_tabled(pbr_ctx* ctx, const pbr_global* g, const pbr_tile* tile,
+                                           const pbr_gbuffer* gb,
+                                           const float* lut_fold, uint32_t lut_res,
+                                           const pbr_half* env_padded, uint32_t env_size, uint32_t env_mips,
+                                           const pbr_cluster* clusters, const pbr_light* lights, int num_lights,
+                                           pbr_half* hdr, uint32_t hdr_pitch, const uint32_t (*rects)[4], uint32_t n_rects,
+                                           const pbr_shade_tables* tables);
 
 pbr_status pbr_deferred_shade_f32(pbr_ctx* ctx, const pbr_global* g, const pbr_tile* tile,
                                   const pbr_gbuffer* gb,
```

Result: faster. 18680 (median of 6 runs) (+1.1%).
